# haotiansun14/rl-rep

Measured on NVIDIA B200. Metric: agent updates/sec, higher is better.
Workload: dtype tf32

## Files before the change

include/rlrep_b200.h:

```cpp
#ifndef RLREP_B200_H_
#define RLREP_B200_H_

#include <stddef.h>
#include <stdint.h>

#ifdef __cplusplus
extern "C" {
#endif

#if defined(__GNUC__)
#define RLREP_EXPORT __attribute__((visibility("default")))
#else
#define RLREP_EXPORT
#endif

#define RLREP_ABI_VERSION 3

RLREP_EXPORT int rlrep_abi_version(void);
RLREP_EXPORT const char* rlrep_last_error(void);


enum { RLREP_ACT_NONE = 0, RLREP_ACT_ELU = 1, RLREP_ACT_RELU = 2, RLREP_ACT_TANH = 3, RLREP_ACT_SIN = 4 };
enum {
  RLREP_DACT_NONE = 0,
  RLREP_DACT_ELU_OUT = 1,
  RLREP_DACT_RELU_OUT = 2,
  RLREP_DACT_TANH_OUT = 3,
  RLREP_DACT_COS_PRE = 4
};

typedef struct rlrep_epilogue {
  const float* bias_dev;
  const float* r1_u_dev;
  const float* r1_v_dev;
  const float* aux_dev;
  float* pre_out_dev;
  int ld_aux;
  int ld_pre;
  int act;
  int dact;
  int accumulate;
  float scale;
} rlrep_epilogue;

RLREP_EXPORT int rlrep_gemm(void* stream, int path, int M, int N, int K, const float* A_dev, int lda, int a_mn,
                            const float* A2_dev, int lda2, int K1, const float* B_dev, int ldb, int b_mn,
                            float* C_dev, int ldc, const rlrep_epilogue* epi, int bn, int split_k, float* ws_dev,
                            size_t ws_floats);

RLREP_EXPORT int rlrep_gemm_bench(void* stream, int path, int M, int N, int K, const float* A_dev, int lda, int a_mn,
                                  const float* B_dev, int ldb, int b_mn, float* C_dev, int ldc,
                                  const rlrep_epilogue* epi, int bn, int split_k, float* ws_dev, size_t ws_floats,
                                  int iters, float* ms_out, int* bn_out, int* split_out);

RLREP_EXPORT int rlrep_gemm_chain_begin(void);
RLREP_EXPORT int rlrep_gemm_chain_add(int M, int N, int K, const float* A_dev, int lda, int a_mn, const float* B_dev,
                                      int ldb, int b_mn, float* C_dev, int ldc, const rlrep_epilogue* epi);
RLREP_EXPORT int rlrep_gemm_chain_run(void* stream, int bn, int split_k, int iters, float* ms_out, int* levels_out);
RLREP_EXPORT int rlrep_gemm_chain_set_debug(unsigned long long* dev);

RLREP_EXPORT int rlrep_gemm_trace(unsigned long long* out16_host);
RLREP_EXPORT int rlrep_gemm_set_debug_buffer(unsigned long long* dev80);

typedef struct rlrep_ring rlrep_ring;

RLREP_EXPORT int rlrep_ring_create(int state_dim, int action_dim, long long capacity, rlrep_ring** out);
RLREP_EXPORT int rlrep_ring_destroy(rlrep_ring* ring);
RLREP_EXPORT int rlrep_ring_layout(const rlrep_ring* ring, int* record_floats, int* off_action, int* off_reward,
                                   int* off_done, int* off_next_state);
RLREP_EXPORT int rlrep_ring_state(const rlrep_ring* ring, long long* size, long long* ptr, long long* capacity);
RLREP_EXPORT int rlrep_ring_add_packed(rlrep_ring* ring, const float* rows_host, int n, void* stream);
RLREP_EXPORT int rlrep_ring_load(rlrep_ring* ring, const void* state_host, const void* action_host,
                                 const void* next_state_host, const void* reward_host, const void* done_host,
                                 long long n, int is_f64, void* stream);
RLREP_EXPORT int rlrep_ring_gather(rlrep_ring* ring, const int64_t* idx_host, int B, float* out_dev, void* stream);

typedef struct rlrep_pixring rlrep_pixring;
RLREP_EXPORT int rlrep_pixring_create(long long capacity, int frame_bytes, int action_dim, int frame_stack, int nstep,
                                      rlrep_pixring** out);
RLREP_EXPORT int rlrep_pixring_destroy(rlrep_pixring* ring);
RLREP_EXPORT int rlrep_pixring_write(rlrep_pixring* ring, long long slot, int copies, const unsigned char* frame_host,
                                     const float* action_host, float reward, float discount, int has_step);
RLREP_EXPORT int rlrep_pixring_flush(rlrep_pixring* ring);
RLREP_EXPORT int rlrep_pixring_gather(rlrep_pixring* ring, const int64_t* idx_host, int n, const float* discount_vec_host,
                                      float next_dis, unsigned char* obs_dev, float* act_dev, float* rew_dev, float* dis_dev,
                                      unsigned char* nobs_dev, unsigned char* sobs_dev);

typedef struct rlrep_agent rlrep_agent;

enum { RLREP_ALG_SAC = 0, RLREP_ALG_CTRLSAC = 1, RLREP_ALG_VLSAC = 2, RLREP_ALG_SPEDERSAC = 3, RLREP_ALG_DIFFSRSAC = 4 };
enum { RLREP_PRECISION_TF32 = 0, RLREP_PRECISION_FP32 = 1 };

typedef struct rlrep_agent_config {
  int alg;
  int state_dim, action_dim, batch_size;
  int hidden_dim, feature_dim, actor_hidden_dim;
  int feature_steps;
  double lr_critic, lr_feature, lr_actor, lr_alpha;
  float discount, tau, feature_tau;
  double alpha;
  int target_update_period, auto_entropy_tuning, use_feature_target;
  int precision;
  int use_cuda_graph;
  int phi_hidden_dim, phi_hidden_depth, mu_hidden_dim, mu_hidden_depth;
  int nabla_mu_hidden_dim, nabla_mu_hidden_depth, num_noise, num_noises;
  float sigma_scale_factor;
} rlrep_agent_config;

RLREP_EXPORT int rlrep_agent_create(const rlrep_agent_config* cfg, void* stream, rlrep_agent** out);

typedef struct rlrep_comm rlrep_comm;
RLREP_EXPORT int rlrep_comm_unique_id(unsigned char* out128);
RLREP_EXPORT int rlrep_comm_create(const unsigned char* id128, int rank, int world, rlrep_comm** out);
RLREP_EXPORT int rlrep_comm_destroy(rlrep_comm* comm);
RLREP_EXPORT int rlrep_comm_info(rlrep_comm* comm, int* rank, int* world, int* nccl_version, long long* collectives);
RLREP_EXPORT int rlrep_agent_create_sharded(const rlrep_agent_config* cfg, rlrep_comm* comm, void* stream,
                                            rlrep_agent** out);
RLREP_EXPORT int rlrep_agent_destroy(rlrep_agent* agent);

RLREP_EXPORT int rlrep_agent_num_tensors(rlrep_agent* agent, int* n);
RLREP_EXPORT int rlrep_agent_tensor_info(rlrep_agent* agent, int i, const char** name, float** ptr_dev, int* rows,
                                         int* cols);
RLREP_EXPORT int rlrep_agent_tensor_read(rlrep_agent* agent, int i, float* out_host);
RLREP_EXPORT int rlrep_agent_tensor_write(rlrep_agent* agent, int i, const float* in_host);
RLREP_EXPORT int rlrep_agent_sync_targets(rlrep_agent* agent);
RLREP_EXPORT int rlrep_agent_get_log_alpha(rlrep_agent* agent, double* log_alpha);
RLREP_EXPORT int rlrep_agent_set_log_alpha(rlrep_agent* agent, double log_alpha);
typedef struct rlrep_optim_state {
  int steps;
  long long t_feature, t_critic, t_actor, t_alpha;
  double log_alpha, log_alpha_m, log_alpha_v;
} rlrep_optim_state;
RLREP_EXPORT int rlrep_agent_get_optim_state(rlrep_agent* agent, rlrep_optim_state* out);
RLREP_EXPORT int rlrep_agent_set_optim_state(rlrep_agent* agent, const rlrep_optim_state* in);
RLREP_EXPORT int rlrep_agent_get_steps(rlrep_agent* agent, int* steps);

RLREP_EXPORT int rlrep_agent_train_counts(rlrep_agent* agent, int* n_idx, int* n_eps, int* n_metrics);
RLREP_EXPORT const char* rlrep_agent_metric_name(rlrep_agent* agent, int i);
RLREP_EXPORT int rlrep_agent_train(rlrep_agent* agent, rlrep_ring* ring, const int64_t* idx_host, int n_idx,
                                   const float* eps_host, int n_eps, float* metrics_host, int n_metrics);
RLREP_EXPORT int rlrep_agent_act(rlrep_agent* agent, const float* state_host, const float* eps_host,
// ... 132 lines not shown
```

rlrep_b200/_lib.py:

```python
from __future__ import annotations

import ctypes as C
from pathlib import Path

_HERE = Path(__file__).resolve().parent
LIB_PATH = _HERE / "librlrep_b200.so"


class RlrepError(RuntimeError):
    pass


class OptimState(C.Structure):
    _fields_ = [("steps", C.c_int), ("t_feature", C.c_longlong), ("t_critic", C.c_longlong), ("t_actor", C.c_longlong),
                ("t_alpha", C.c_longlong), ("log_alpha", C.c_double), ("log_alpha_m", C.c_double),
                ("log_alpha_v", C.c_double)]


class AgentConfig(C.Structure):
    _fields_ = [
        ("alg", C.c_int), ("state_dim", C.c_int), ("action_dim", C.c_int), ("batch_size", C.c_int),
        ("hidden_dim", C.c_int), ("feature_dim", C.c_int), ("actor_hidden_dim", C.c_int), ("feature_steps", C.c_int),
        ("lr_critic", C.c_double), ("lr_feature", C.c_double), ("lr_actor", C.c_double), ("lr_alpha", C.c_double),
        ("discount", C.c_float), ("tau", C.c_float), ("feature_tau", C.c_float), ("alpha", C.c_double),
        ("target_update_period", C.c_int), ("auto_entropy_tuning", C.c_int), ("use_feature_target", C.c_int),
        ("precision", C.c_int), ("use_cuda_graph", C.c_int),
        ("phi_hidden_dim", C.c_int), ("phi_hidden_depth", C.c_int), ("mu_hidden_dim", C.c_int),
        ("mu_hidden_depth", C.c_int), ("nabla_mu_hidden_dim", C.c_int), ("nabla_mu_hidden_depth", C.c_int),
        ("num_noise", C.c_int), ("num_noises", C.c_int), ("sigma_scale_factor", C.c_float),
    ]


ALG = {"sac": 0, "ctrlsac": 1, "vlsac": 2, "spedersac": 3, "diffsrsac": 4}
PRECISION = {"tf32": 0, "fp32": 1}


class Epilogue(C.Structure):
    _fields_ = [
        ("bias", C.c_void_p), ("r1_u", C.c_void_p), ("r1_v", C.c_void_p), ("aux", C.c_void_p),
        ("pre_out", C.c_void_p), ("ld_aux", C.c_int), ("ld_pre", C.c_int), ("act", C.c_int),
        ("dact", C.c_int), ("accumulate", C.c_int), ("scale", C.c_float),
    ]


ACT = {"none": 0, "elu": 1, "relu": 2, "tanh": 3, "sin": 4}
DACT = {"none": 0, "elu_out": 1, "relu_out": 2, "tanh_out": 3, "cos_pre": 4}

_lib = None


def load() -> C.CDLL:
    global _lib
    if _lib is not None:
        return _lib
    if not LIB_PATH.exists():
        raise RlrepError(
            f"{LIB_PATH} not found: build it with `python -m rlrep_b200.build` (needs nvcc). "
            "rlrep_b200 has no CPU or PyTorch fallback.")
    lib = C.CDLL(str(LIB_PATH))
    lib.rlrep_last_error.restype = C.c_char_p
    lib.rlrep_abi_version.restype = C.c_int
    _declare(lib)
    _lib = lib
    return lib


def _declare(lib: C.CDLL) -> None:
    vp, i, f, sz = C.c_void_p, C.c_int, C.c_float, C.c_size_t
    sigs = {
        "rlrep_gemm": [vp, i, i, i, i, vp, i, i, vp, i, i, vp, i, i, vp, i, C.POINTER(Epilogue), i, i, vp, sz],
        "rlrep_gemm_bench": [vp, i, i, i, i, vp, i, i, vp, i, i, vp, i, C.POINTER(Epilogue), i, i, vp, sz, i,
                             C.POINTER(C.c_float), C.POINTER(C.c_int), C.POINTER(C.c_int)],
        "rlrep_gemm_trace": [vp],
        "rlrep_gemm_chain_begin": [],
        "rlrep_gemm_chain_set_debug": [vp],
        "rlrep_gemm_chain_add": [i, i, i, vp, i, i, vp, i, i, vp, i, C.POINTER(Epilogue)],
        "rlrep_gemm_chain_run": [vp, i, i, i, C.POINTER(C.c_float), C.POINTER(C.c_int)],
        "rlrep_ring_create": [i, i, C.c_longlong, C.POINTER(vp)],
        "rlrep_ring_destroy": [vp],
        "rlrep_ring_layout": [vp] + [C.POINTER(i)] * 5,
        "rlrep_ring_state": [vp] + [C.POINTER(C.c_longlong)] * 3,
        "rlrep_ring_add_packed": [vp, vp, i, vp],
        "rlrep_ring_load": [vp, vp, vp, vp, vp, vp, C.c_longlong, i, vp],
        "rlrep_ring_gather": [vp, vp, i, vp, vp],
        "rlrep_agent_create": [C.POINTER(AgentConfig), vp, C.POINTER(vp)],
        "rlrep_agent_destroy": [vp],
        "rlrep_conv_encoder_create": [i, i, i, i, vp, C.POINTER(vp)],
        "rlrep_conv_encoder_destroy": [vp],
        "rlrep_conv_encoder_read": [vp, i, i, vp],
        "rlrep_conv_encoder_write": [vp, i, i, vp],
        "rlrep_conv_encoder_forward": [vp, vp, vp, vp],
        "rlrep_conv_encoder_backward": [vp, vp],
        "rlrep_conv_encoder_feature_dim": [vp, C.POINTER(i)],
        "rlrep_conv_encoder_forward_pitched": [vp, vp, vp, vp, i, i],
        "rlrep_conv_encoder_backward_pitched": [vp, vp, i],
        "rlrep_conv_encoder_read_map": [vp, i, i, vp],
        "rlrep_conv_decoder_create": [i, i, i, vp, C.POINTER(vp)],
        "rlrep_conv_decoder_destroy": [vp],
        "rlrep_conv_decoder_read": [vp, i, i, vp],
        "rlrep_conv_decoder_write": [vp, i, i, vp],
        "rlrep_conv_decoder_forward": [vp, vp, i],
        "rlrep_conv_decoder_l1_loss": [vp, vp, f, vp],
        "rlrep_conv_decoder_mse_sum_loss": [vp, vp, vp, f, vp],
        "rlrep_conv_decoder_backward": [vp, vp, i],
        "rlrep_conv_decoder_read_map": [vp, i, i, vp],
        "rlrep_drq_create": [vp, vp, C.POINTER(vp)],
        "rlrep_drq_destroy": [vp],
        "rlrep_drq_num_tensors": [vp, C.POINTER(i)],
        "rlrep_drq_tensor_info": [vp, i, C.POINTER(C.c_char_p), C.POINTER(vp), C.POINTER(i), C.POINTER(i)],
        "rlrep_drq_tensor_read": [vp, i, vp],
        "rlrep_drq_tensor_write": [vp, i, vp],
        "rlrep_drq_sync_targets": [vp],
        "rlrep_drq_update": [vp, vp, vp, vp, vp, vp, vp, vp, C.c_float, vp],
        "rlrep_drq_last_launches": [vp, C.POINTER(i)],
        "rlrep_drq_act": [vp, vp, vp, C.c_float, vp],
        "rlrep_drq_act_batch": [vp, vp, vp, C.c_float, i, vp],
        "rlrep_drq_update_resident": [vp, i, C.c_float, C.POINTER(C.c_float)],
        "rlrep_drq_profile_update": [vp, C.c_float, i, C.POINTER(C.c_char_p), C.POINTER(C.c_float), C.POINTER(C.c_double),
                                     C.POINTER(C.c_double), C.POINTER(i)],
        "rlrep_gemm_set_debug_buffer": [vp],
        "rlrep_ldiff_create": [vp, vp, C.POINTER(vp)],
        "rlrep_ldiff_destroy": [vp],
        "rlrep_ldiff_num_tensors": [vp, C.POINTER(i)],
        "rlrep_ldiff_tensor_info": [vp, i, C.POINTER(C.c_char_p), C.POINTER(vp), C.POINTER(i), C.POINTER(i)],
        "rlrep_ldiff_tensor_read": [vp, i, vp],
        "rlrep_ldiff_tensor_write": [vp, i, vp],
        "rlrep_ldiff_sync_targets": [vp],
        "rlrep_ldiff_update": [vp, vp, vp],
        "rlrep_ldiff_update_resident": [vp, i, C.c_float, C.POINTER(C.c_float)],
        "rlrep_ldiff_profile_update": [vp, C.c_float, i, C.POINTER(C.c_char_p), C.POINTER(C.c_float),
                                       C.POINTER(C.c_double), C.POINTER(C.c_double), C.POINTER(i)],
        "rlrep_ldiff_last_launches": [vp, C.POINTER(i)],
        "rlrep_mulv_create": [vp, vp, C.POINTER(vp)],
        "rlrep_mulv_destroy": [vp],
        "rlrep_mulv_num_tensors": [vp, C.POINTER(i)],
        "rlrep_mulv_tensor_info": [vp, i, C.POINTER(C.c_char_p), C.POINTER(vp), C.POINTER(i), C.POINTER(i)],
        "rlrep_mulv_tensor_read": [vp, i, vp],
        "rlrep_mulv_tensor_write": [vp, i, vp],
        "rlrep_mulv_sync_targets": [vp],
        "rlrep_mulv_update": [vp, vp, vp, vp, vp, vp, vp, vp, vp, vp, vp, C.c_float, vp],
        "rlrep_mulv_last_launches": [vp, C.POINTER(i)],
        "rlrep_mulv_act": [vp, vp, vp, C.c_float, vp],
        "rlrep_mulv_act_batch": [vp, vp, vp, C.c_float, i, vp],
        "rlrep_mulv_update_resident": [vp, i, C.c_float, C.POINTER(C.c_float)],
        "rlrep_mulv_profile_update": [vp, C.c_float, i, C.POINTER(C.c_char_p), C.POINTER(C.c_float), C.POINTER(C.c_double),
                                      C.POINTER(C.c_double), C.POINTER(i)],
        "rlrep_comm_unique_id": [vp],
        "rlrep_comm_create": [vp, i, i, C.POINTER(vp)],
        "rlrep_comm_destroy": [vp],
        "rlrep_comm_info": [vp, C.POINTER(i), C.POINTER(i), C.POINTER(i), C.POINTER(C.c_longlong)],
        "rlrep_agent_create_sharded": [C.POINTER(AgentConfig), vp, vp, C.POINTER(vp)],
        "rlrep_agent_num_tensors": [vp, C.POINTER(i)],
        "rlrep_agent_tensor_info": [vp, i, C.POINTER(C.c_char_p), C.POINTER(vp), C.POINTER(i), C.POINTER(i)],
        "rlrep_agent_tensor_read": [vp, i, vp],
        "rlrep_agent_tensor_write": [vp, i, vp],
        "rlrep_agent_sync_targets": [vp],
        "rlrep_agent_get_log_alpha": [vp, C.POINTER(C.c_double)],
        "rlrep_agent_set_log_alpha": [vp, C.c_double],
        "rlrep_agent_get_steps": [vp, C.POINTER(i)],
        "rlrep_agent_get_optim_state": [vp, C.POINTER(OptimState)],
        "rlrep_agent_set_optim_state": [vp, C.POINTER(OptimState)],
        "rlrep_agent_train_counts": [vp, C.POINTER(i), C.POINTER(i), C.POINTER(i)],
        "rlrep_agent_train": [vp, vp, vp, i, vp, i, vp, i],
        "rlrep_agent_act": [vp, vp, vp, vp],
        "rlrep_pixring_create": [C.c_longlong, i, i, i, i, C.POINTER(vp)],
        "rlrep_pixring_destroy": [vp],
        "rlrep_pixring_write": [vp, C.c_longlong, i, vp, vp, C.c_float, C.c_float, i],
        "rlrep_pixring_flush": [vp],
        "rlrep_pixring_gather": [vp, vp, i, vp, C.c_float, vp, vp, vp, vp, vp, vp],
        "rlrep_agent_act_batch": [vp, vp, vp, i, vp],
        "rlrep_agent_last_launches": [vp, C.POINTER(i)],
        "rlrep_agent_graph_stats": [vp, C.POINTER(i), C.POINTER(i)],
        "rlrep_agent_train_resident": [vp, vp, vp, vp, i, C.POINTER(C.c_float)],
        "rlrep_agent_profile_train": [vp, vp, vp, vp, i, C.POINTER(C.c_char_p), C.POINTER(C.c_float),
                                      C.POINTER(C.c_double), C.POINTER(C.c_double), C.POINTER(i)],
    }
    lib.rlrep_agent_metric_name.argtypes = [vp, i]
    lib.rlrep_agent_metric_name.restype = C.c_char_p
    for name, argtypes in sigs.items():
        fn = getattr(lib, name)
        fn.argtypes = argtypes
        fn.restype = C.c_int


def check(rc: int) -> None:
    if rc != 0:
        msg = load().rlrep_last_error()
        raise RlrepError(msg.decode() if msg else f"rlrep call failed with code {rc}")


def current_stream_ptr() -> int:
    import torch
    return torch.cuda.current_stream().cuda_stream


def make_epilogue(bias=None, r1=None, aux=None, pre_out=None, act="none", dact="none", accumulate=False,
                  scale=1.0) -> Epilogue:
    e = Epilogue()
    e.bias = bias.data_ptr() if bias is not None else None
    if r1 is not None:
        e.r1_u, e.r1_v = r1[0].data_ptr(), r1[1].data_ptr()
    if aux is not None:
        e.aux, e.ld_aux = aux.data_ptr(), aux.stride(0)
    if pre_out is not None:
        e.pre_out, e.ld_pre = pre_out.data_ptr(), pre_out.stride(0)
    e.act, e.dact = ACT[act], DACT[dact]
    e.accumulate = int(accumulate)
    e.scale = scale
    return e


def gemm(A, B, C_out, *, a_mn=False, b_mn=False, path="tc", epi: Epilogue | None = None, A2=None, bn=0, split_k=0,
         ws=None):
    lib = load()
    M = A.shape[1] if a_mn else A.shape[0]
    K = A.shape[0] if a_mn else A.shape[1]
    N = B.shape[1] if b_mn else B.shape[0]
    K1 = K
    if A2 is not None:
        K += A2.shape[1]
    assert (B.shape[0] if b_mn else B.shape[1]) == K
    epi = epi or make_epilogue()
    rc = lib.rlrep_gemm(current_stream_ptr(), 0 if path == "tc" else 1, M, N, K, A.data_ptr(), A.stride(0), int(a_mn),
                        A2.data_ptr() if A2 is not None else None, A2.stride(0) if A2 is not None else 0, K1,
                        B.data_ptr(), B.stride(0), int(b_mn), C_out.data_ptr(), C_out.stride(0), C.byref(epi), bn,
                        split_k, ws.data_ptr() if ws is not None else None, ws.numel() if ws is not None else 0)
    check(rc)
    return C_out


def gemm_chain(specs, *, bn=0, split_k=0, iters=1):
    lib = load()
    check(lib.rlrep_gemm_chain_begin())
    keep = []
    for A, B, C_out, kw in specs:
        a_mn, b_mn = bool(kw.get("a_mn", False)), bool(kw.get("b_mn", False))
        M = A.shape[1] if a_mn else A.shape[0]
        K = A.shape[0] if a_mn else A.shape[1]
        N = B.shape[1] if b_mn else B.shape[0]
        assert (B.shape[0] if b_mn else B.shape[1]) == K
        epi = kw.get("epi") or make_epilogue()
        keep.append(epi)
        check(lib.rlrep_gemm_chain_add(M, N, K, A.data_ptr(), A.stride(0), int(a_mn), B.data_ptr(), B.stride(0), int(b_mn),
                                       C_out.data_ptr(), C_out.stride(0), C.byref(epi)))
    ms, levels = C.c_float(), C.c_int()
    check(lib.rlrep_gemm_chain_run(current_stream_ptr(), bn, split_k, iters, C.byref(ms), C.byref(levels)))
    return ms.value, levels.value


def gemm_bench(A, B, C_out, *, a_mn=False, b_mn=False, path="tc", epi=None, bn=0, split_k=0, ws=None, iters=50):
    lib = load()
    M = A.shape[1] if a_mn else A.shape[0]
    K = A.shape[0] if a_mn else A.shape[1]
    N = B.shape[1] if b_mn else B.shape[0]
    epi = epi or make_epilogue()
    ms, bno, so = C.c_float(), C.c_int(), C.c_int()
    rc = lib.rlrep_gemm_bench(current_stream_ptr(), 0 if path == "tc" else 1, M, N, K, A.data_ptr(), A.stride(0),
                              int(a_mn), B.data_ptr(), B.stride(0), int(b_mn), C_out.data_ptr(), C_out.stride(0),
                              C.byref(epi), bn, split_k, ws.data_ptr() if ws is not None else None,
                              ws.numel() if ws is not None else 0, iters, C.byref(ms), C.byref(bno), C.byref(so))
    check(rc)
    return ms.value, bno.value, so.value
```

rlrep_b200/csrc/agent.cuh:

```cuda
#pragma once
#include <cuda_runtime.h>

#include <cstdint>
#include <cstring>
#include <functional>
#include <memory>
#include <string>
#include <unordered_map>
#include <vector>

#include "common.cuh"
#include "gemm.cuh"
#include "gemm_chain.cuh"
#include "kernels.cuh"

namespace rlrep {

class DeviceArena {
 public:
  DeviceArena() = default;
  DeviceArena(const DeviceArena&) = delete;
  DeviceArena& operator=(const DeviceArena&) = delete;
  ~DeviceArena() { release(); }
  template <typename T>
// ... 91 lines not shown
inline int round_up32(int x) { return (x + 31) & ~31; }

inline LinearSlot add_linear(ParamGroup& g, const std::string& name, int out, int in, bool pad = true) {
  LinearSlot s;
  s.out = out;
  s.in = in;
  s.ld = pad ? round_up32(in) : in;
  s.out_alloc = pad ? round_up32(out) : out;
  s.w_off = g.add(name + ".weight", out, in, s.ld, s.out_alloc);
  s.b_off = g.add(name + ".bias", out, 1, 1, s.out_alloc);
  return s;
}

inline LinearSlot add_stacked(ParamGroup& g, const std::string& a, int out_a, const std::string& b, int out_b, int in) {
  RLREP_CHECK(in % 32 == 0, "stacked heads need an input width that is a multiple of 32");
  LinearSlot s;
  s.out = out_a + out_b;
  s.in = in;
  s.ld = in;
  s.out_alloc = round_up32(s.out);
  s.w_off = g.add(a + ".weight", out_a, in);
  g.add(b + ".weight", out_b, in, in, s.out_alloc - out_a);
  s.b_off = g.add(a + ".bias", out_a, 1, 1, out_a, true);
  g.add(b + ".bias", out_b, 1, 1, s.out_alloc - out_a, true);
  g.align4();
  return s;
}

struct RecordLayout {
  int R, off_a, off_r, off_d, off_s2;
  static RecordLayout of(int S, int A) {
    RecordLayout l;
    l.off_a = S;
    l.off_r = S + A;
    l.off_d = S + A + 1;
    l.off_s2 = (S + A + 2 + 3) & ~3;
    l.R = (l.off_s2 + S + 3) & ~3;
    return l;
  }
};

class Ring {
 public:
  Ring(int state_dim, int action_dim, long long capacity);
  ~Ring();
  Ring(const Ring&) = delete;
  Ring& operator=(const Ring&) = delete;

  int S, A, R;
  int off_a, off_r, off_d, off_s2;
  long long capacity, size = 0, ptr = 0;
  float* data = nullptr;
  const unsigned long long generation;

  void add_packed(const float* rows_host, int n, cudaStream_t s);
  void load_columns(const void* state, const void* action, const void* next_state, const void* reward,
                    const void* done, long long n, int is_f64, cudaStream_t s);
  void gather_from_host_idx(const long long* idx_host, int B, float* out_dev, cudaStream_t s);

 private:
  float* stage_host_ = nullptr;
  float* stage_dev_ = nullptr;
  long long* idx_host_ = nullptr;
  long long* idx_dev_ = nullptr;
  size_t stage_rows_ = 0;
  int idx_cap_ = 0;
};

enum Precision : int { PREC_TF32 = 0, PREC_FP32 = 1 };

class GemmRunner {
 public:
  void init(Precision prec, size_t ws_floats);
  ~GemmRunner();
  void run(const GemmArgs& a, cudaStream_t s);
  bool run_compact(GemmArgs a, int wp, int ho, cudaStream_t s);
  bool compact_supported(GemmArgs a, int wp, int ho);
  void set_sm_share(double share) { sm_share_ = share; }

  bool chains_enabled() const { return prec_ == PREC_TF32; }
  void begin_chain(cudaStream_t s);
  void end_chain();
  bool recording() const { return recording_; }

 private:
  void flush_chain();
  bool recording_ = false;
  cudaStream_t chain_stream_ = nullptr;
  std::vector<GemmArgs> pending_;
  std::vector<std::unique_ptr<GemmChain>> chains_;
  Precision prec_ = PREC_TF32;
  double sm_share_ = 1.0;
  float* ws_ = nullptr;
  size_t ws_floats_ = 0;
  float* kg_ws_ = nullptr;
  size_t kg_ws_floats_ = 0;
  std::unordered_map<std::string, TcGemmPlan> plans_;
};

struct Mat {
  const float* p = nullptr;
  int ld = 0;
};
void linear_fwd(GemmRunner& g, cudaStream_t s, int rows, Mat x, const Linear& l, int act, float* y, int ldy,
                Mat x2 = Mat(), int k1 = 0, float* pre_out = nullptr);
void linear_dgrad(GemmRunner& g, cudaStream_t s, int rows, Mat dy, const Linear& l, int dact, Mat aux, float* dx,
                  int lddx, int col0 = 0, int n_cols = -1);
void linear_wgrad(GemmRunner& g, cudaStream_t s, int rows, Mat dy, Mat x, const Linear& l, Mat x2 = Mat(), int k1 = 0,
                  bool bias_grad = true);
inline ColJob bias_job(int rows, Mat dy, const Linear& l) {
  ColJob j;
  j.X = dy.p; j.ld = dy.ld; j.rows = rows; j.cols = l.out; j.u = nullptr; j.out = l.db;
  return j;
}

class GraphReplay {
 public:
  ~GraphReplay() { reset(); }
  void reset();
  void run(cudaStream_t s, bool enabled, const std::function<void()>& body);
  bool captured() const { return exec_ != nullptr; }
  bool stats(int* kernel_nodes, int* programmatic_edges) const;

 private:
  int calls_ = 0;
  cudaGraph_t graph_ = nullptr;
  cudaGraphExec_t exec_ = nullptr;
};

struct AgentConfig {
  int alg = 0;
  int state_dim = 0, action_dim = 0, batch = 256;
  int hidden_dim = 256, feature_dim = 256, actor_hidden_dim = 256;
  int k_feat = 0;
  double lr = 3e-4, lr_feat = 1e-4, lr_actor = 1e-4, lr_alpha = 1e-4;
  float discount = 0.99f, tau = 0.005f, feature_tau = 0.005f;
  double alpha0 = 0.1;
  int target_update_period = 2, learn_alpha = 1, use_feature_target = 1;
  int precision = PREC_TF32;
  int use_graph = 1;
  int phi_hidden_dim = 0, phi_hidden_depth = 0, mu_hidden_dim = 0, mu_hidden_depth = 0;
  int nabla_hidden_dim = 0, nabla_hidden_depth = 0, num_noise = 20, num_noises = 1000;
  float sigma_scale = 0.449f;
};

class Agent {
 public:
  virtual ~Agent() = default;
  virtual void train(Ring& ring, const long long* idx_host, int n_idx, const float* eps_host, int n_eps,
                     float* metrics_host, int n_metrics) = 0;
  virtual float train_resident(Ring& ring, const long long* idx_host, const float* eps_host, int n_steps) = 0;
  virtual std::vector<ProfileEntry> profile_train(Ring& ring, const long long* idx_host, const float* eps_host) = 0;
  virtual int idx_per_train() const = 0;
  virtual int eps_per_train() const = 0;
  virtual const std::vector<std::string>& metric_names() const = 0;
  virtual std::vector<ParamGroup*> groups() = 0;
  virtual void act(const float* state_host, const float* eps_host, float* action_host) = 0;
  virtual void act_batch(const float* states_host, const float* eps_host, int rows, float* actions_host) = 0;
  virtual void sync_targets_from_params() = 0;
  virtual bool graph_stats(int* kernel_nodes, int* programmatic_edges) const = 0;

  AgentConfig cfg;
  cudaStream_t stream = nullptr;
  Control* ctl = nullptr;
  int last_launches = 0;
};

std::unique_ptr<Agent> make_sac_agent(const AgentConfig& cfg, cudaStream_t s);
std::unique_ptr<Agent> make_ctrlsac_agent(const AgentConfig& cfg, cudaStream_t s);
std::unique_ptr<Agent> make_vlsac_agent(const AgentConfig& cfg, cudaStream_t s);
std::unique_ptr<Agent> make_spedersac_agent(const AgentConfig& cfg, cudaStream_t s);
std::unique_ptr<Agent> make_diffsrsac_agent(const AgentConfig& cfg, cudaStream_t s);
// ... 5 lines not shown
```

rlrep_b200/csrc/agent_ctrlsac.cu:

```cuda
#include "agent_base.cuh"

namespace rlrep {

namespace {

class CtrlSacAgent final : public SacBase {
 public:
  CtrlSacAgent(const AgentConfig& c, cudaStream_t s) : SacBase(c, s) {
    H_ = c.hidden_dim;
    D_ = c.feature_dim;
    K_ = c.k_feat;
    RLREP_CHECK(K_ >= 1 && K_ <= kMaxFeatureSteps, "extra_feature_steps out of range");
    const RecordLayout probe_layout = RecordLayout::of(S_, A_);
    off_r_ = probe_layout.off_r;
    off_d_ = probe_layout.off_d;
    off_s2_ = probe_layout.off_s2;
    plan_common(K_ * B_, 2 * B_ * A_, probe_layout.R);

    feat_g_.name = "feature";
    p1_ = add_linear(feat_g_, "phi.l1", H_, S_ + A_);
    p2_ = add_linear(feat_g_, "phi.l2", H_, H_);
    p3_ = add_linear(feat_g_, "phi.l3", D_, H_);
    feat_g_.n_target = feat_g_.n;
    feat_g_.target_prefix_from = "phi.";
// ... 167 lines not shown
      gemm_.run(a, s1);
    }
    wait_for(w1, mark(s1));
    gemm_.set_sm_share(wshare);
    linear_wgrad(gemm_, w1, B_, Mat{dzmu_, D_}, Mat{g2_, H_}, n3, Mat(), 0, false);
    gemm_.set_sm_share(share);
    linear_dgrad(gemm_, s1, B_, Mat{dzmu_, D_}, n3, DACT_ELU_OUT, Mat{g2_, H_}, dg2_, H_);
    wait_for(w1, mark(s1));
    gemm_.set_sm_share(wshare);
    linear_wgrad(gemm_, w1, B_, Mat{dg2_, H_}, Mat{g1_, H_}, n2, Mat(), 0, false);
    gemm_.set_sm_share(share);
    linear_dgrad(gemm_, s1, B_, Mat{dg2_, H_}, n2, DACT_ELU_OUT, Mat{g1_, H_}, dg1_, H_);
    linear_wgrad(gemm_, s1, B_, Mat{dg1_, H_}, s2(), n1, Mat(), 0, false);
    wait_for(w1, mark(s1));
    {
      ColJob jobs[3] = {bias_job(B_, Mat{dzmu_, D_}, n3), bias_job(B_, Mat{dg2_, H_}, n2),
                        bias_job(B_, Mat{dg1_, H_}, n1)};
      launch_colreduce_multi(jobs, 3, w1);
    }
    join_aux(0, s0);
    join_aux(1, s0);
    join();
    launch_adam_polyak(feat_g_.p, feat_g_.g, feat_g_.m, feat_g_.v, feat_g_.n, &ctl->feat[k],
                       cfg.use_feature_target ? feat_g_.target : nullptr, feat_g_.n_target, cfg.feature_tau, nullptr,
                       s0);
  }

  void feature_step_chained(int k, Ring& ring) {
    const Linear l1 = p1_.view(feat_g_), l2 = p2_.view(feat_g_), l3 = p3_.view(feat_g_);
    const Linear n1 = m1_.view(feat_g_), n2 = m2_.view(feat_g_), n3 = m3_.view(feat_g_);
    const Linear th = th_.view(feat_g_);
    const float inv_b = 1.f / (float)B_;
    cudaStream_t s0 = stream;
    launch_gather(ring.data, R_ / 4, idx_dev_ + (size_t)k * B_, B_, batch_, s0);
    gemm_.begin_chain(s0);
    phi_forward(s0, sa(), Mat(), 0, zphi_, h1_, h2_);
    linear_fwd(gemm_, s0, B_, s2(), n1, ACT_ELU, g1_, H_);
    linear_fwd(gemm_, s0, B_, Mat{g1_, H_}, n2, ACT_ELU, g2_, H_);
    linear_fwd(gemm_, s0, B_, Mat{g2_, H_}, n3, ACT_TANH, zmu_, D_);
    {
      GemmArgs a;
      a.M = B_; a.N = B_; a.K = D_;
      a.A = zphi_; a.lda = D_;
      a.B = zmu_; a.ldb = D_;
      a.C = logits_; a.ldc = B_;
      gemm_.run(a, s0);
    }
    if (k == K_ - 1) {
      actor_trunk(s2(), 1, s0);
      actor_trunk(Mat{batch_, R_}, 0, s0);
    }
    gemm_.end_chain();
    launch_contrastive_head(logits_, B_, B_, B_, 0, inv_b, zphi_, D_, D_, th.W, th.b, reward(), R_, loss_rows_, rpred_, drp_,
                            metrics_dev_ + 0, head_ctr_, s0);
    gemm_.begin_chain(s0);
    {
      GemmArgs a;
      a.M = B_; a.N = D_; a.K = B_;
      a.A = logits_; a.lda = B_;
      a.B = zmu_; a.ldb = D_; a.b_mn = true;
      a.C = dzphi_; a.ldc = D_;
      a.epi.r1_u = drp_; a.epi.r1_v = th.W;
      gemm_.run(a, s0);
    }
    {
      GemmArgs a;
      a.M = B_; a.N = D_; a.K = B_;
      a.A = logits_; a.lda = B_; a.a_mn = true;
      a.B = zphi_; a.ldb = D_; a.b_mn = true;
      a.C = dzmu_; a.ldc = D_;
      a.epi.dact = DACT_TANH_OUT; a.epi.aux = zmu_; a.epi.ld_aux = D_;
      gemm_.run(a, s0);
    }
    linear_dgrad(gemm_, s0, B_, Mat{dzphi_, D_}, l3, DACT_ELU_OUT, Mat{h2_, H_}, dh2_, H_);
    linear_dgrad(gemm_, s0, B_, Mat{dzmu_, D_}, n3, DACT_ELU_OUT, Mat{g2_, H_}, dg2_, H_);
    linear_wgrad(gemm_, s0, B_, Mat{dzphi_, D_}, Mat{h2_, H_}, l3, Mat(), 0, false);
    linear_wgrad(gemm_, s0, B_, Mat{dzmu_, D_}, Mat{g2_, H_}, n3, Mat(), 0, false);
    linear_dgrad(gemm_, s0, B_, Mat{dh2_, H_}, l2, DACT_ELU_OUT, Mat{h1_, H_}, dh1_, H_);
    linear_dgrad(gemm_, s0, B_, Mat{dg2_, H_}, n2, DACT_ELU_OUT, Mat{g1_, H_}, dg1_, H_);
    linear_wgrad(gemm_, s0, B_, Mat{dh2_, H_}, Mat{h1_, H_}, l2, Mat(), 0, false);
    linear_wgrad(gemm_, s0, B_, Mat{dg2_, H_}, Mat{g1_, H_}, n2, Mat(), 0, false);
    linear_wgrad(gemm_, s0, B_, Mat{dh1_, H_}, sa(), l1, Mat(), 0, false);
    linear_wgrad(gemm_, s0, B_, Mat{dg1_, H_}, s2(), n1, Mat(), 0, false);
    gemm_.end_chain();
    {
      ColJob jobs[8] = {bias_job(B_, Mat{dzphi_, D_}, l3), bias_job(B_, Mat{dh2_, H_}, l2),
                        bias_job(B_, Mat{dh1_, H_}, l1), ColJob{zphi_, drp_, th.dW, D_, B_, D_},
                        ColJob{drp_, nullptr, th.db, 1, B_, 1},
                        bias_job(B_, Mat{dzmu_, D_}, n3), bias_job(B_, Mat{dg2_, H_}, n2),
                        bias_job(B_, Mat{dg1_, H_}, n1)};
      launch_colreduce_multi(jobs, 8, s0);
    }
    launch_adam_polyak(feat_g_.p, feat_g_.g, feat_g_.m, feat_g_.v, feat_g_.n, &ctl->feat[k],
                       cfg.use_feature_target ? feat_g_.target : nullptr, feat_g_.n_target, cfg.feature_tau, nullptr,
                       s0);
  }

  void critic_step_chained() {
    cudaStream_t s0 = stream;
    const float* eps_next = eps_dev_;
    const float* eps_pi = eps_dev_ + (size_t)B_ * A_;
    const Linear l14t = c14_.view(crit_g_, true), l14 = c14_.view(crit_g_), l2 = c2_.view(crit_g_), l5 = c5_.view(crit_g_);
    const Linear l2t = c2_.view(crit_g_, true), l5t = c5_.view(crit_g_, true);
    actor_sample_cat_pair(s2(), eps_next, logp2_, Mat{batch_, R_}, eps_pi, s0);
    const Mat s2a{cat_next_, LDSA_}, spi{cat_pi_, LDSA_};
    gemm_.begin_chain(s0);
    phi_forward(s0, s2a, Mat(), 0, zmu_, h1_, h2_);
    linear_fwd(gemm_, s0, B_, Mat{zmu_, D_}, l14t, ACT_ELU, hid_t_, 2 * H_);
    phi_forward(s0, sa(), Mat(), 0, zphi_, hb1_, hb2_);
    linear_fwd(gemm_, s0, B_, Mat{zphi_, D_}, l14, ACT_ELU, hid_, 2 * H_);
    phi_forward(s0, spi, Mat(), 0, zpi_, hc1_, hc2_);
    gemm_.end_chain();
    {
      CriticHeadArgs a;
      a.hid_t = hid_t_; a.hid = hid_; a.ldh = 2 * H_; a.H = H_; a.B = B_;
      a.w2t = l2t.W; a.b2t = l2t.b; a.w5t = l5t.W; a.b5t = l5t.b;
      a.w2 = l2.W; a.b2 = l2.b; a.w5 = l5.W; a.b5 = l5.b;
      a.reward = reward(); a.done = done(); a.ld_rd = R_;
      a.logp2 = logp2_; a.gamma = cfg.discount; a.c = ctl;
      a.nq1 = nq1_; a.nq2 = nq2_; a.q1 = q1_; a.q2 = q2_; a.dq1 = dq1_; a.dq2 = dq2_;
      a.dhid = dhid_; a.ld_dh = 2 * H_;
      a.metrics = metrics_dev_ + 3;
      a.counter = head_ctr_ + 1;
      launch_critic_td_head(a, s0);
    }
    {
      ColJob jobs[5] = {ColJob{hid_, dq1_, l2.dW, 2 * H_, B_, H_}, ColJob{dq1_, nullptr, l2.db, 1, B_, 1},
                        ColJob{hid_ + H_, dq2_, l5.dW, 2 * H_, B_, H_}, ColJob{dq2_, nullptr, l5.db, 1, B_, 1},
                        bias_job(B_, Mat{dhid_, 2 * H_}, l14)};
      launch_colreduce_multi(jobs, 5, s0);
    }
    linear_wgrad(gemm_, s0, B_, Mat{dhid_, 2 * H_}, Mat{zphi_, D_}, l14, Mat(), 0, false);
    launch_adam_polyak(crit_g_.p, crit_g_.g, crit_g_.m, crit_g_.v, crit_g_.n, &ctl->critic, crit_g_.target,
                       crit_g_.n_target, cfg.tau, &ctl->polyak_critic, s0);
  }

  void actor_step_chained() {
    const float* eps = eps_dev_ + (size_t)B_ * A_;
    const Linear l14 = c14_.view(crit_g_);
    const Linear l1 = p1_.view(feat_g_), l2 = p2_.view(feat_g_), l3 = p3_.view(feat_g_);
    {
      const Linear c2 = c2_.view(crit_g_), c5 = c5_.view(crit_g_);
      linear_fwd(gemm_, stream, B_, Mat{zpi_, D_}, l14, ACT_ELU, hid_, 2 * H_);
      ActorHeadArgs a;
      a.hid = hid_; a.ldh = 2 * H_; a.H = H_; a.B = B_;
      a.w2 = c2.W; a.b2 = c2.b; a.w5 = c5.W; a.b5 = c5.b;
      a.logp = logp_; a.target_entropy = (float)(-A_); a.learn_alpha = cfg.learn_alpha; a.c = ctl;
      a.q1 = q1_; a.q2 = q2_; a.dq1 = dq1_; a.dq2 = dq2_;
      a.dhid = dhid_; a.ld_dh = 2 * H_;
      a.dlogp_scalar = dlogp_;
      a.metrics = metrics_dev_ + 7;
      a.counter = head_ctr_ + 2;
      launch_actor_head(a, stream);
    }
    gemm_.begin_chain(stream);
    linear_dgrad(gemm_, stream, B_, Mat{dhid_, 2 * H_}, l14, DACT_NONE, Mat(), dzphi_, D_);
    linear_dgrad(gemm_, stream, B_, Mat{dzphi_, D_}, l3, DACT_ELU_OUT, Mat{hc2_, H_}, dh2_, H_);
    linear_dgrad(gemm_, stream, B_, Mat{dh2_, H_}, l2, DACT_ELU_OUT, Mat{hc1_, H_}, dh1_, H_);
    dgrad_to_action(Mat{dh1_, H_}, l1);
    gemm_.end_chain();
    actor_backward_chained(Mat{batch_, R_}, eps);
    actor_adam();
  }

  void critic_forward(cudaStream_t s, const float* z, bool target, float* hid, float* q1, float* q2) {
    const Linear l14 = c14_.view(crit_g_, target), l2 = c2_.view(crit_g_, target), l5 = c5_.view(crit_g_, target);
    linear_fwd(gemm_, s, B_, Mat{z, D_}, l14, ACT_ELU, hid, 2 * H_);
    launch_rowdot_pair(RowDotJob{hid, l2.W, l2.b, q1, 2 * H_, H_}, RowDotJob{hid + H_, l5.W, l5.b, q2, 2 * H_, H_}, B_, s);
  }
  void critic_heads_backward_to_hidden() {
    const Linear l2 = c2_.view(crit_g_), l5 = c5_.view(crit_g_);
    launch_outer_dact(dq1_, l2.W, B_, H_, hid_, 2 * H_, DACT_ELU_OUT, dhid_, 2 * H_, stream);
    launch_outer_dact(dq2_, l5.W, B_, H_, hid_ + H_, 2 * H_, DACT_ELU_OUT, dhid_ + H_, 2 * H_, stream);
  }

  void critic_step() {
    const float* eps = eps_dev_;
    cudaStream_t s0 = stream, s1 = side();
// ... 66 lines not shown
```

rlrep_b200/csrc/capi.cu:

```cuda
#include <algorithm>
#include <cmath>
#include <memory>
#include <string>
#include <vector>

#include "agent.cuh"
#include "gemm_chain.cuh"
#include "comm.cuh"
#include "common.cuh"
#include "conv.cuh"
#include "deconv.cuh"
#include "drq.cuh"
#include "layout.cuh"
#include "mulv.cuh"
#include "pixel_replay.cuh"
#include "ldiffsr.cuh"
#include "gemm.cuh"
#include "rlrep_b200.h"

namespace rlrep {
namespace {
thread_local std::string g_last_error;
}
void set_last_error(const std::string& msg) { g_last_error = msg; }
// ... 37 lines not shown
  int prev = -1;
  explicit DeviceGuard(int want) {
    if (want < 0) return;
    int cur = 0;
    if (cudaGetDevice(&cur) == cudaSuccess && cur != want && cudaSetDevice(want) == cudaSuccess) prev = cur;
  }
  ~DeviceGuard() {
    if (prev >= 0) cudaSetDevice(prev);
  }
};
#define RLREP_API_BEGIN_ON(h) RLREP_API_BEGIN DeviceGuard _device_guard((h) != nullptr ? (h)->device : -1);

struct rlrep_ring {
  int device = current_device();
  std::unique_ptr<Ring> impl;
};

struct rlrep_comm {
  int device = current_device();
  std::unique_ptr<Comm> impl;
};

struct TensorRef {
  std::string name;
  float* ptr;
  int rows, cols, ld;
};

struct rlrep_agent {
  int device = current_device();
  std::unique_ptr<Agent> impl;
  std::vector<TensorRef> tensors;
  cudaStream_t owned_stream = nullptr;
};

static void index_tensors(rlrep_agent* a) {
  a->tensors.clear();
  for (ParamGroup* g : a->impl->groups()) {
    for (const ParamTensor& t : g->tensors) a->tensors.push_back({t.name, g->p + t.offset, t.rows, t.cols, t.ld});
    if (g->m && g->v)
      for (const ParamTensor& t : g->tensors) {
        a->tensors.push_back({"optim.m/" + t.name, g->m + t.offset, t.rows, t.cols, t.ld});
        a->tensors.push_back({"optim.v/" + t.name, g->v + t.offset, t.rows, t.cols, t.ld});
      }
    if (g->target) {
      for (const ParamTensor& t : g->tensors) {
        if (t.offset >= g->n_target) continue;
        if (t.name.compare(0, g->target_prefix_from.size(), g->target_prefix_from) != 0) continue;
        a->tensors.push_back({g->target_prefix_to + t.name.substr(g->target_prefix_from.size()), g->target + t.offset,
                              t.rows, t.cols, t.ld});
      }
    }
  }
}

extern "C" {

int rlrep_abi_version(void) { return RLREP_ABI_VERSION; }
const char* rlrep_last_error(void) { return get_last_error(); }

int rlrep_gemm(void* stream, int path, int M, int N, int K, const float* A, int lda, int a_mn, const float* A2,
               int lda2, int K1, const float* B, int ldb, int b_mn, float* C, int ldc, const rlrep_epilogue* epi,
               int bn, int split_k, float* ws, size_t ws_floats) {
  RLREP_API_BEGIN
  GemmArgs g;
  g.M = M; g.N = N; g.K = K;
  g.A = A; g.lda = lda; g.a_mn = a_mn != 0;
  g.A2 = A2; g.lda2 = lda2; g.K1 = K1;
  g.B = B; g.ldb = ldb; g.b_mn = b_mn != 0;
  g.C = C; g.ldc = ldc;
  g.epi = to_epilogue(epi);
  cudaStream_t st = static_cast<cudaStream_t>(stream);
  if (path == 0) {
    TcGemmPlan p = make_tc_plan(g, bn, split_k, ws, ws_floats);
    launch_tc(p, st);
  } else {
    launch_simt(g, st);
  }
  RLREP_API_END
}

namespace {
thread_local std::vector<GemmArgs> g_chain_seq;
}

int rlrep_gemm_chain_set_debug(unsigned long long* dev) {
  RLREP_API_BEGIN
  set_chain_debug_buffer(dev);
  RLREP_API_END
}

int rlrep_gemm_chain_begin(void) {
  RLREP_API_BEGIN
  g_chain_seq.clear();
  RLREP_API_END
}

int rlrep_gemm_chain_add(int M, int N, int K, const float* A, int lda, int a_mn, const float* B, int ldb, int b_mn,
                         float* C, int ldc, const rlrep_epilogue* epi) {
  RLREP_API_BEGIN
  GemmArgs g;
  g.M = M; g.N = N; g.K = K;
  g.A = A; g.lda = lda; g.a_mn = a_mn != 0;
  g.B = B; g.ldb = ldb; g.b_mn = b_mn != 0;
  g.C = C; g.ldc = ldc;
  g.epi = to_epilogue(epi);
  RLREP_CHECK(chain_eligible(g), "operands violate the tensor-core path's constraints (see rlrep_gemm, path 0)");
  g_chain_seq.push_back(g);
  RLREP_API_END
}

int rlrep_gemm_chain_run(void* stream, int bn, int split_k, int iters, float* ms_out, int* levels_out) {
  RLREP_API_BEGIN
  RLREP_CHECK(!g_chain_seq.empty() && iters >= 1, "empty chain");
  cudaStream_t st = static_cast<cudaStream_t>(stream);
  GemmChain chain;
  chain.build(g_chain_seq, bn, split_k);
  if (levels_out) *levels_out = chain.levels();
  cudaEvent_t e0, e1;
  RLREP_CUDA(cudaEventCreate(&e0));
  RLREP_CUDA(cudaEventCreate(&e1));
  chain.launch(st);
  RLREP_CUDA(cudaEventRecord(e0, st));
  for (int i = 1; i < iters; ++i) chain.launch(st);
  RLREP_CUDA(cudaEventRecord(e1, st));
  RLREP_CUDA(cudaStreamSynchronize(st));
  float ms = 0.f;
  RLREP_CUDA(cudaEventElapsedTime(&ms, e0, e1));
  cudaEventDestroy(e0);
  cudaEventDestroy(e1);
  if (ms_out) *ms_out = iters > 1 ? ms / (iters - 1) : 0.f;
  g_chain_seq.clear();
  RLREP_API_END
}

int rlrep_gemm_bench(void* stream, int path, int M, int N, int K, const float* A, int lda, int a_mn, const float* B,
                     int ldb, int b_mn, float* C, int ldc, const rlrep_epilogue* epi, int bn, int split_k, float* ws,
                     size_t ws_floats, int iters, float* ms_out, int* bn_out, int* split_out) {
  RLREP_API_BEGIN
  GemmArgs g;
  g.M = M; g.N = N; g.K = K;
  g.A = A; g.lda = lda; g.a_mn = a_mn != 0;
  g.B = B; g.ldb = ldb; g.b_mn = b_mn != 0;
  g.C = C; g.ldc = ldc;
  g.epi = to_epilogue(epi);
  cudaStream_t st = static_cast<cudaStream_t>(stream);
  cudaEvent_t e0, e1;
  RLREP_CUDA(cudaEventCreate(&e0));
  RLREP_CUDA(cudaEventCreate(&e1));
  TcGemmPlan p;
  if (path == 0) {
    p = make_tc_plan(g, bn, split_k, ws, ws_floats);
    if (bn_out) *bn_out = p.bn;
    if (split_out) *split_out = p.split_k;
  }
  auto launch_once = [&](cudaStream_t s) {
    if (path == 0) launch_tc(p, s);
    else if (path == 1) launch_simt(g, s);
    else if (path == 2) null_kernel<<<M, 128, 0, s>>>(C);
    else {
      cudaLaunchConfig_t cfg = {};
      cfg.gridDim = dim3(M);
      cfg.blockDim = dim3(128);
      cfg.stream = s;
      cudaLaunchAttribute at[1];
      at[0].id = cudaLaunchAttributeProgrammaticStreamSerialization;
      at[0].val.programmaticStreamSerializationAllowed = 1;
      cfg.attrs = at;
      cfg.numAttrs = 1;
      RLREP_CUDA(cudaLaunchKernelEx(&cfg, null_pdl_kernel, C));
    }
  };
  for (int i = 0; i < 3; ++i) launch_once(st);
  cudaStream_t cs;
  RLREP_CUDA(cudaStreamCreateWithFlags(&cs, cudaStreamNonBlocking));
  cudaGraph_t graph;
  cudaGraphExec_t exec;
  RLREP_CUDA(cudaStreamSynchronize(st));
  RLREP_CUDA(cudaStreamBeginCapture(cs, cudaStreamCaptureModeThreadLocal));
  for (int i = 0; i < iters; ++i) launch_once(cs);
  RLREP_CUDA(cudaStreamEndCapture(cs, &graph));
  RLREP_CUDA(cudaGraphInstantiate(&exec, graph, 0));
  RLREP_CUDA(cudaGraphLaunch(exec, cs));
  RLREP_CUDA(cudaEventRecord(e0, cs));
  RLREP_CUDA(cudaGraphLaunch(exec, cs));
  RLREP_CUDA(cudaEventRecord(e1, cs));
  RLREP_CUDA(cudaStreamSynchronize(cs));
  cudaGraphExecDestroy(exec);
  cudaGraphDestroy(graph);
  cudaStreamDestroy(cs);
  RLREP_CUDA(cudaEventSynchronize(e1));
  float ms = 0.f;
  RLREP_CUDA(cudaEventElapsedTime(&ms, e0, e1));
  *ms_out = ms / iters;
  cudaEventDestroy(e0);
  cudaEventDestroy(e1);
  RLREP_API_END
}

int rlrep_gemm_set_debug_buffer(unsigned long long* dev80) {
  RLREP_API_BEGIN
  set_gemm_debug_buffer(dev80);
  RLREP_API_END
}
int rlrep_gemm_trace(unsigned long long* out16_host) {
  RLREP_API_BEGIN
  RLREP_CUDA(cudaDeviceSynchronize());
  read_gemm_trace(out16_host);
  RLREP_API_END
}

int rlrep_ring_create(int state_dim, int action_dim, long long capacity, rlrep_ring** out) {
  RLREP_API_BEGIN
  RLREP_CHECK(out != nullptr, "null out pointer");
  std::unique_ptr<rlrep_ring> r(new rlrep_ring);
// ... 986 lines not shown
```

rlrep_b200/csrc/gemm_chain.cu:

```cuda
#include <algorithm>
#include <cmath>
#include <cstdlib>
#include <cstring>

#include "common.cuh"
#include "gemm_chain.cuh"
#include "ptx.cuh"

namespace rlrep {

namespace {

constexpr int kThreads = 320;
constexpr int kEpiWarps = 8;
constexpr int kStages = 6;
constexpr int kCW = 16;
constexpr int kTwPitch = kCW + 4;
constexpr int kMaxBn = 128;
constexpr int kBM = 128, kBK = 32;
constexpr int kABytes = kBM * kBK * 4;
constexpr int kStageBytes = kABytes + kMaxBn * kBK * 4;
constexpr int kTbufFloats = kEpiWarps * 32 * kTwPitch;
constexpr int kSub = 4, kCtrStride = 32;
constexpr int kDbgItems = 16, kDbgEvents = 10;
// ... 57 lines not shown
  const float e = __expf(n) - 1.f;
  const float r = n < -0.34657359f ? e : p;
  return x > 0.f ? x : r;
}

__device__ __forceinline__ bool aligned16(const void* p) { return (reinterpret_cast<uintptr_t>(p) & 15) == 0; }

__device__ __forceinline__ float chain_epilogue_scalar(const Epilogue& e, float acc, int m, int n, const float* cptr) {
  float v = acc * e.scale;
  if (e.r1_u) v = fmaf(__ldcg(e.r1_u + m), __ldcg(e.r1_v + n), v);
  if (e.bias) v += __ldg(e.bias + n);
  if (e.pre_out) e.pre_out[(size_t)m * e.ld_pre + n] = v;
  v = apply_act(v, e.act);
  if (e.dact != DACT_NONE) v *= apply_dact(__ldcg(e.aux + (size_t)m * e.ld_aux + n), e.dact);
  if (e.accumulate) v += __ldcg(cptr);
  return v;
}

struct ChunkOperands {
  float4 bias, r1v;
  float4 aux[4];
  float r1u[4];
};
__device__ __forceinline__ void chunk_prefetch(ChunkOperands& o, const Epilogue& epi, int M, int m_base, int gn0, int lane) {
  const int piece = lane & 3, rsub = lane >> 2;
  const int on = gn0 + 4 * piece;
  o.bias = make_float4(0.f, 0.f, 0.f, 0.f);
  o.r1v = make_float4(0.f, 0.f, 0.f, 0.f);
  if (epi.bias) o.bias = __ldg(reinterpret_cast<const float4*>(epi.bias + on));
  if (epi.r1_u) o.r1v = __ldcg(reinterpret_cast<const float4*>(epi.r1_v + on));
#pragma unroll
  for (int r4 = 0; r4 < 4; ++r4) {
    const int om = m_base + r4 * 8 + rsub;
    o.aux[r4] = make_float4(0.f, 0.f, 0.f, 0.f);
    o.r1u[r4] = 0.f;
    if (om < M) {
      if (epi.dact != DACT_NONE) o.aux[r4] = __ldcg(reinterpret_cast<const float4*>(epi.aux + (size_t)om * epi.ld_aux + on));
      if (epi.r1_u) o.r1u[r4] = __ldcg(epi.r1_u + om);
    }
  }
}

template <int ACT, int DACT>
__device__ __forceinline__ void chain_store_rows(const Epilogue& epi, const ChunkOperands& o, const float* tw,
                                                 float* __restrict__ C, int ldc, int M, int m_base, int gn0, int lane) {
  const int piece = lane & 3, rsub = lane >> 2;
  const int on = gn0 + 4 * piece;
#pragma unroll
  for (int r4 = 0; r4 < 4; ++r4) {
    const int r = r4 * 8 + rsub;
    const int om = m_base + r;
    if (om < M) {
      const float4 a4 = *reinterpret_cast<const float4*>(tw + r * kTwPitch + 4 * piece);
      float v[4] = {a4.x * epi.scale, a4.y * epi.scale, a4.z * epi.scale, a4.w * epi.scale};
      if (epi.r1_u) {
        const float u = o.r1u[r4];
        v[0] = fmaf(u, o.r1v.x, v[0]); v[1] = fmaf(u, o.r1v.y, v[1]); v[2] = fmaf(u, o.r1v.z, v[2]); v[3] = fmaf(u, o.r1v.w, v[3]);
      }
      v[0] += o.bias.x; v[1] += o.bias.y; v[2] += o.bias.z; v[3] += o.bias.w;
      if (epi.pre_out)
        *reinterpret_cast<float4*>(epi.pre_out + (size_t)om * epi.ld_pre + on) = make_float4(v[0], v[1], v[2], v[3]);
      if constexpr (ACT != ACT_NONE) {
#pragma unroll
        for (int e = 0; e < 4; ++e) v[e] = ACT == ACT_ELU ? elu_fast(v[e]) : apply_act(v[e], ACT < 0 ? epi.act : ACT);
      }
      if constexpr (DACT != DACT_NONE) {
        const int dact = DACT < 0 ? epi.dact : DACT;
        if (dact != DACT_NONE) {
          const float4 x = o.aux[r4];
          v[0] *= apply_dact(x.x, dact); v[1] *= apply_dact(x.y, dact); v[2] *= apply_dact(x.z, dact); v[3] *= apply_dact(x.w, dact);
        }
      }
      float4* cp = reinterpret_cast<float4*>(C + (size_t)om * ldc + on);
      if (epi.accumulate) {
        const float4 c0 = __ldcg(cp);
        v[0] += c0.x; v[1] += c0.y; v[2] += c0.z; v[3] += c0.w;
      }
      *cp = make_float4(v[0], v[1], v[2], v[3]);
    }
  }
}

__global__ void __launch_bounds__(kThreads, 1)
gemm_chain_kernel(const ChainGemmDesc* __restrict__ gemms, const ChainTask* __restrict__ tasks,
                  const int* __restrict__ task_begin, unsigned* __restrict__ done, unsigned* __restrict__ exit_ctr,
                  int n_gemms, unsigned long long* __restrict__ dbg) {
  auto stamp = [&](int item, int ev) {
    if (dbg != nullptr && item < kDbgItems) {
      unsigned long long t;
      asm volatile("mov.u64 %0, %%globaltimer;" : "=l"(t)::"memory");
      dbg[((size_t)blockIdx.x * kDbgItems + item) * kDbgEvents + ev] = t;
    }
  };
  if (threadIdx.x == 0) stamp(kDbgItems - 1, 2);
  extern __shared__ uint8_t smem_raw[];
  uint8_t* smem = reinterpret_cast<uint8_t*>((reinterpret_cast<uintptr_t>(smem_raw) + 1023) & ~uintptr_t(1023));
  uint64_t* full_bar = reinterpret_cast<uint64_t*>(smem + kStages * kStageBytes);
  uint64_t* empty_bar = full_bar + 8;
  uint64_t* acc_full = empty_bar + 8;
  uint64_t* acc_empty = acc_full + 2;
  uint32_t* tmem_slot = reinterpret_cast<uint32_t*>(acc_empty + 2);
  volatile unsigned* arrival = reinterpret_cast<volatile unsigned*>(tmem_slot + 1);
  float* tbuf = reinterpret_cast<float*>(smem + kStages * kStageBytes + 256);

  const int warp = threadIdx.x >> 5, lane = threadIdx.x & 31;
  const int t_begin = task_begin[blockIdx.x], t_end = task_begin[blockIdx.x + 1];

  if (threadIdx.x == 0) {
    for (int s = 0; s < kStages; ++s) {
      ptx::mbar_init(&full_bar[s], 1);
      ptx::mbar_init(&empty_bar[s], 1);
    }
    for (int a = 0; a < 2; ++a) {
      ptx::mbar_init(&acc_full[a], 1);
      ptx::mbar_init(&acc_empty[a], kEpiWarps);
    }
    ptx::fence_mbar_init();
  }
  if (warp == 1) {
    ptx::tmem_alloc(tmem_slot, 2 * kMaxBn);
    ptx::tmem_relinquish();
  }
  ptx::tc_fence_before_sync();
  __syncthreads();
  ptx::tc_fence_after_sync();
  const uint32_t tmem_base = *tmem_slot;
  ptx::pdl_wait();

  if (warp == 0) {
    if (lane == 0) {
      int it = 0, last_gemm = -1;
      for (int t = t_begin; t < t_end; ++t) {
        const ChainTask tk = tasks[t];
        const ChainGemmDesc* g = gemms + tk.gemm;
        const int n_deps = g->n_deps;
        const int bn = g->bn, a_mn = g->a_mn, b_mn = g->b_mn;
        const int m0 = (tk.tile % g->tiles_m) * kBM, n0 = (tk.tile / g->tiles_m) * bn;
        const int kb0 = tk.split * g->kb_per_split, kb1 = min(g->nkb, kb0 + g->kb_per_split);
        int dep_id[kChainMaxDeps], dep_tiles[kChainMaxDeps];
#pragma unroll
        for (int d = 0; d < kChainMaxDeps; ++d) {
          dep_id[d] = d < n_deps ? g->dep[d] : 0;
          dep_tiles[d] = d < n_deps ? (int)g->dep_target[d] : 0;
        }
        if (tk.gemm != last_gemm) {
          fence_tensormap_acquire(&g->tmA);
          fence_tensormap_acquire(&g->tmB);
          last_gemm = tk.gemm;
        }
        stamp(t - t_begin, 0);
        if (dbg != nullptr && t - t_begin < kDbgItems)
          dbg[((size_t)blockIdx.x * kDbgItems + (t - t_begin)) * kDbgEvents + 8] =
              (unsigned long long)tk.gemm | ((unsigned long long)tk.tile << 16) | ((unsigned long long)tk.split << 40);
#pragma unroll
        for (int d = 0; d < kChainMaxDeps; ++d)
          if (d < n_deps) wait_counter(done, dep_id[d], dep_tiles[d]);
        if (n_deps > 0) {
          fence_acquire_gpu();
          fence_proxy_async_global();
        }
        stamp(t - t_begin, 1);
        const uint32_t tx = kABytes + bn * kBK * 4;
        for (int kb = kb0; kb < kb1; ++kb, ++it) {
          const int s = it % kStages;
          ptx::mbar_wait(&empty_bar[s], ((it / kStages) & 1) ^ 1);
          ptx::mbar_arrive_expect_tx(&full_bar[s], tx);
          uint8_t* a_dst = smem + s * kStageBytes;
          uint8_t* b_dst = a_dst + kABytes;
          const int k0 = kb * kBK;
          if (!a_mn) ptx::tma_load_2d(a_dst, &g->tmA, &full_bar[s], k0, m0);
          else ptx::tma_load_3d(a_dst, &g->tmA, &full_bar[s], 0, k0, m0 / 32);
          if (!b_mn) ptx::tma_load_2d(b_dst, &g->tmB, &full_bar[s], k0, n0);
          else ptx::tma_load_3d(b_dst, &g->tmB, &full_bar[s], 0, k0, n0 / 32);
        }
        stamp(t - t_begin, 2);
      }
    }
  } else if (warp == 1) {
    if (ptx::elect_one()) {
      int it = 0, tc = 0;
      for (int t = t_begin; t < t_end; ++t, ++tc) {
        const ChainTask tk = tasks[t];
        const ChainGemmDesc* g = gemms + tk.gemm;
        const int bn = g->bn, a_mn = g->a_mn, b_mn = g->b_mn;
        const int kb0 = tk.split * g->kb_per_split, kb1 = min(g->nkb, kb0 + g->kb_per_split);
        const uint32_t idesc = ptx::make_idesc_tf32(kBM, bn, a_mn != 0, b_mn != 0);
        const int acc = tc & 1;
        ptx::mbar_wait(&acc_empty[acc], ((tc >> 1) & 1) ^ 1);
        ptx::tc_fence_after_sync();
        const uint32_t d_tmem = tmem_base + acc * kMaxBn;
        for (int kb = kb0; kb < kb1; ++kb, ++it) {
          const int s = it % kStages;
          ptx::mbar_wait(&full_bar[s], (it / kStages) & 1);
          if (kb == kb0) stamp(t - t_begin, 3);
          ptx::tc_fence_after_sync();
          const uint32_t a_addr = ptx::smem_u32(smem + s * kStageBytes);
          const uint32_t b_addr = a_addr + kABytes;
#pragma unroll
          for (int k = 0; k < kBK / 8; ++k) {
            const uint64_t adesc = a_mn ? ptx::make_smem_desc(a_addr + k * 1024, 4096, 512, 1)
                                        : ptx::make_smem_desc(a_addr + k * 32, 16, 1024, 2);
            const uint64_t bdesc = b_mn ? ptx::make_smem_desc(b_addr + k * 1024, 4096, 512, 1)
                                        : ptx::make_smem_desc(b_addr + k * 32, 16, 1024, 2);
            ptx::mma_tf32_ss(d_tmem, adesc, bdesc, idesc, (kb > kb0 || k > 0) ? 1u : 0u);
          }
          ptx::mma_commit(&empty_bar[s]);
        }
        ptx::mma_commit(&acc_full[acc]);
        stamp(t - t_begin, 4);
      }
    }
  } else {
    const int q = warp & 3, half = (warp - 2) >> 2;
    float* tw = tbuf + (warp - 2) * (32 * kTwPitch);
    int tc = 0;
    for (int t = t_begin; t < t_end; ++t, ++tc) {
      const ChainTask tk = tasks[t];
      const ChainGemmDesc* g = gemms + tk.gemm;
      const Epilogue epi = g->epi;
      const int bn = g->bn, M = g->M, N = g->N, ldc = g->ldc, split_k = g->split_k;
      float* __restrict__ C = g->C;
      float* __restrict__ ws = g->ws;
      unsigned* __restrict__ tile_ctr = g->tile_ctr;
      const int m0 = (tk.tile % g->tiles_m) * kBM, n0 = (tk.tile / g->tiles_m) * bn;
      const int chunks = bn / kCW;
      const int acc = tc & 1;
      const uint32_t t_acc = tmem_base + (static_cast<uint32_t>(32 * q) << 16) + acc * kMaxBn;
      const int row = 32 * q + lane;
      ptx::mbar_wait(&acc_full[acc], (tc >> 1) & 1);
      if (threadIdx.x == 64) stamp(t - t_begin, 5);
      ptx::tc_fence_after_sync();

      bool final = true;
      const size_t part_floats = (size_t)kBM * bn;
      float* ws_tile = split_k > 1 ? ws + (size_t)tk.tile * split_k * part_floats : nullptr;
      const bool dist = split_k > 1 && g->dist != 0;
      int c_first = half, c_step = 2;
      if (split_k > 1) {
        float* part = ws_tile + (size_t)tk.split * part_floats;
#pragma unroll 1
        for (int c = half; c < chunks; c += 2) {
          if (dist && c % split_k == tk.split) continue;
          uint32_t v[kCW];
          ptx::tmem_ld_32x32b_x16(t_acc + c * kCW, v);
          ptx::tmem_ld_wait();
#pragma unroll
          for (int j = 0; j < kCW / 4; ++j)
            __stcg(reinterpret_cast<float4*>(part + ((size_t)(c * (kCW / 4) + j) * kBM + row) * 4),
                   make_float4(__uint_as_float(v[4 * j]), __uint_as_float(v[4 * j + 1]), __uint_as_float(v[4 * j + 2]),
                               __uint_as_float(v[4 * j + 3])));
        }
        epilogue_bar();
        if (threadIdx.x == 64) {
          unsigned* ctr = tile_ctr + tk.tile;
          const unsigned old = atom_add_acq_rel(ctr, 1u);
          if (dist) {
            if (old + 1 < (unsigned)split_k) {
              unsigned long long t0 = 0;
              unsigned spins = 0;
              while (ld_relaxed(ctr) < (unsigned)split_k) {
                __nanosleep(20);
                if ((++spins & 0xfff) == 0) {
                  unsigned long long now;
                  asm volatile("mov.u64 %0, %%globaltimer;" : "=l"(now));
                  if (t0 == 0) t0 = now;
                  else if (now - t0 > 2000000000ull) __trap();
                }
              }
              fence_acquire_gpu();
            }
          } else if (old == (unsigned)(split_k - 1)) {
            *ctr = 0;
          }
          *arrival = old;
          stamp(t - t_begin, 6);
        }
        epilogue_bar();
        final = dist || *arrival == (unsigned)(split_k - 1);
        if (dist) {
          c_first = tk.split + split_k * half;
          c_step = 2 * split_k;
        }
      }
      if (final) {
        const bool use_aux = epi.dact != DACT_NONE;
        const bool vec_ok = (ldc & 3) == 0 && aligned16(C) && (N & 3) == 0 &&
                            (!use_aux || ((epi.ld_aux & 3) == 0 && aligned16(epi.aux))) &&
                            (!epi.pre_out || ((epi.ld_pre & 3) == 0 && aligned16(epi.pre_out))) &&
                            (!epi.bias || aligned16(epi.bias)) && (!epi.r1_v || aligned16(epi.r1_v));
#pragma unroll 1
        for (int c = c_first; c < chunks; c += c_step) {
          const int gn0 = n0 + c * kCW;
          const bool fast = vec_ok && gn0 + kCW <= N;
          ChunkOperands ops;
          if (fast) chunk_prefetch(ops, epi, M, m0 + 32 * q, gn0, lane);
          float a[kCW];
          if (split_k == 1) {
            uint32_t v[kCW];
            ptx::tmem_ld_32x32b_x16(t_acc + c * kCW, v);
            ptx::tmem_ld_wait();
// ... 3 lines not shown
            const float* base = ws_tile + ((size_t)(c * (kCW / 4)) * kBM + row) * 4;
            float4 nxt[kCW / 4];
            const int s_first = tk.split == 0 ? 1 : 0;
#pragma unroll
            for (int j = 0; j < kCW / 4; ++j)
              nxt[j] = __ldcg(reinterpret_cast<const float4*>(base + (size_t)s_first * part_floats + (size_t)j * kBM * 4));
#pragma unroll 1
            for (int s = 0; s < split_k; ++s) {
              if (s == tk.split) {
                uint32_t v[kCW];
                ptx::tmem_ld_32x32b_x16(t_acc + c * kCW, v);
                ptx::tmem_ld_wait();
                if (s == 0) {
#pragma unroll
                  for (int e = 0; e < kCW; ++e) a[e] = __uint_as_float(v[e]);
                } else {
#pragma unroll
                  for (int e = 0; e < kCW; ++e) a[e] += __uint_as_float(v[e]);
                }
                continue;
              }
              float4 cur[kCW / 4];
#pragma unroll
              for (int j = 0; j < kCW / 4; ++j) cur[j] = nxt[j];
              int s2 = s + 1;
              if (s2 == tk.split) ++s2;
              if (s2 < split_k) {
#pragma unroll
                for (int j = 0; j < kCW / 4; ++j)
                  nxt[j] = __ldcg(reinterpret_cast<const float4*>(base + (size_t)s2 * part_floats + (size_t)j * kBM * 4));
              }
              if (s == 0) {
#pragma unroll
                for (int j = 0; j < kCW / 4; ++j) { a[4 * j] = cur[j].x; a[4 * j + 1] = cur[j].y; a[4 * j + 2] = cur[j].z; a[4 * j + 3] = cur[j].w; }
              } else {
#pragma unroll
                for (int j = 0; j < kCW / 4; ++j) { a[4 * j] += cur[j].x; a[4 * j + 1] += cur[j].y; a[4 * j + 2] += cur[j].z; a[4 * j + 3] += cur[j].w; }
              }
            }
          }
#pragma unroll
          for (int j = 0; j < kCW / 4; ++j)
            *reinterpret_cast<float4*>(tw + lane * kTwPitch + 4 * j) = make_float4(a[4 * j], a[4 * j + 1], a[4 * j + 2], a[4 * j + 3]);
          __syncwarp();
          if (fast) {
#define RLREP_CSTORE(A, D) chain_store_rows<A, D>(epi, ops, tw, C, ldc, M, m0 + 32 * q, gn0, lane)
            RLREP_EPILOGUE_SWITCH(epi, RLREP_CSTORE);
#undef RLREP_CSTORE
          } else if (gn0 < N) {
            const int piece = lane & 3, rsub = lane >> 2;
#pragma unroll 1
            for (int r4 = 0; r4 < 4; ++r4) {
              const int r = r4 * 8 + rsub, om = m0 + 32 * q + r;
              if (om >= M) continue;
#pragma unroll 1
              for (int e = 0; e < 4; ++e) {
                const int on = gn0 + 4 * piece + e;
                if (on < N) {
                  float* cp = C + (size_t)om * ldc + on;
                  *cp = chain_epilogue_scalar(epi, tw[r * kTwPitch + 4 * piece + e], om, on, cp);
                }
              }
            }
          }
          __syncwarp();
        }
        if (threadIdx.x == 64) stamp(t - t_begin, 9);
        epilogue_bar();
        if (threadIdx.x == 64) {
          fence_proxy_async_global();
          const int pub = dist ? tk.tile * split_k + tk.split : tk.tile;
          red_release_add(done + ((size_t)tk.gemm * kSub + (pub % kSub)) * kCtrStride, 1u);
          stamp(t - t_begin, 7);
          if (dist) {
            unsigned* ctr = tile_ctr + tk.tile;
            if (atomicAdd(ctr, 1u) == (unsigned)(2 * split_k - 1)) *ctr = 0;
          }
        }
      }
      ptx::tc_fence_before_sync();
      __syncwarp();
      if (lane == 0) ptx::mbar_arrive(&acc_empty[acc]);
    }
  }
  ptx::pdl_launch_dependents();
  ptx::tc_fence_before_sync();
  __syncthreads();
  if (warp == 1) ptx::tmem_dealloc(tmem_base, 2 * kMaxBn);
  if (threadIdx.x == 0) {
    const unsigned old = atom_add_acq_rel(exit_ctr, 1u);
    if (old == gridDim.x - 1) {
      for (int i = 0; i < n_gemms * kSub; ++i) done[(size_t)i * kCtrStride] = 0;
      *exit_ctr = 0;
      __threadfence();
    }
    stamp(kDbgItems - 1, 3);
  }
}

struct Range {
  uintptr_t lo = 0, hi = 0;
  bool overlaps(const Range& o) const { return lo < o.hi && o.lo < hi && lo != hi && o.lo != o.hi; }
};
Range range_of(const float* p, long long rows, long long ld, long long cols) {
  Range r;
  if (p == nullptr || rows <= 0 || cols <= 0) return r;
  r.lo = reinterpret_cast<uintptr_t>(p);
  r.hi = r.lo + (size_t)((rows - 1) * ld + cols) * sizeof(float);
  return r;
}
struct Footprint {
  std::vector<Range> reads, writes;
};
Footprint footprint(const GemmArgs& a) {
  Footprint f;
  f.reads.push_back(a.a_mn ? range_of(a.A, a.K, a.lda, a.M) : range_of(a.A, a.M, a.lda, a.K));
  f.reads.push_back(a.b_mn ? range_of(a.B, a.K, a.ldb, a.N) : range_of(a.B, a.N, a.ldb, a.K));
  f.reads.push_back(range_of(a.epi.bias, 1, 0, a.N));
  f.reads.push_back(range_of(a.epi.r1_u, 1, 0, a.M));
  f.reads.push_back(range_of(a.epi.r1_v, 1, 0, a.N));
  if (a.epi.dact != DACT_NONE) f.reads.push_back(range_of(a.epi.aux, a.M, a.epi.ld_aux, a.N));
  f.writes.push_back(range_of(a.C, a.M, a.ldc, a.N));
  if (a.epi.accumulate) f.reads.push_back(f.writes.back());
  f.writes.push_back(range_of(a.epi.pre_out, a.M, a.epi.ld_pre, a.N));
  return f;
}
bool conflicts(const Footprint& earlier, const Footprint& later) {
  for (const Range& w : earlier.writes) {
    for (const Range& r : later.reads)
      if (w.overlaps(r)) return true;
    for (const Range& r : later.writes)
      if (w.overlaps(r)) return true;
  }
  for (const Range& w : later.writes)
    for (const Range& r : earlier.reads)
      if (w.overlaps(r)) return true;
  return false;
}

unsigned long long* g_chain_dbg = nullptr;

int env_int(const char* name, int dflt) {
  const char* e = std::getenv(name);
  return e ? std::atoi(e) : dflt;
}

bool dist_possible(int bn, int split) { return split > 1 && (bn / kCW) % split == 0; }
double plan_cost(int tiles, int nkb, int bn, int split, int share, bool dist) {
  const int kb_per = ceil_div(nkb, split);
  const double kb_bytes = kABytes + bn * kBK * 4;
  const double waves = std::ceil((double)tiles * split / share);
  const double stream = waves * kb_per * kb_bytes / 150e3;
  const double chip = (double)tiles * split * kb_per * kb_bytes / 12e6;
  if (dist) {
    return 1.5 + std::max(stream, chip) + waves * (0.25 * ceil_div(bn, 64) + 1.0 + 1.0 * ceil_div(bn / split, 64)) +
           0.1 * (split - 1);
  }
  double t = 1.5 + std::max(stream, chip) + waves * 1.0 * ceil_div(bn, 64);
  if (split > 1) t += 1.5 + 0.3 * (split - 1) * ceil_div(bn, 64);
  return t;
}

}

void set_chain_debug_buffer(unsigned long long* dev) { g_chain_dbg = dev; }

bool chain_eligible(const GemmArgs& a) {
  return tc_eligible(a) && a.conv_w == 0 && a.M >= 32 && a.N >= 32 && a.K >= 8;
}

GemmChain::~GemmChain() {
  if (dev_) cudaFree(dev_);
}

bool GemmChain::matches(const std::vector<GemmArgs>& seq) const {
  if (seq.size() != seq_.size()) return false;
  for (size_t i = 0; i < seq.size(); ++i) {
    const GemmArgs &x = seq[i], &y = seq_[i];
    if (x.M != y.M || x.N != y.N || x.K != y.K || x.A != y.A || x.B != y.B || x.C != y.C || x.lda != y.lda ||
        x.ldb != y.ldb || x.ldc != y.ldc || x.a_mn != y.a_mn || x.b_mn != y.b_mn || x.epi.bias != y.epi.bias ||
        x.epi.r1_u != y.epi.r1_u || x.epi.r1_v != y.epi.r1_v || x.epi.aux != y.epi.aux || x.epi.pre_out != y.epi.pre_out ||
        x.epi.ld_aux != y.epi.ld_aux || x.epi.ld_pre != y.epi.ld_pre || x.epi.act != y.epi.act || x.epi.dact != y.epi.dact ||
        x.epi.accumulate != y.epi.accumulate || x.epi.scale != y.epi.scale)
      return false;
  }
  return true;
}

void GemmChain::build(const std::vector<GemmArgs>& seq, int force_bn, int force_split) {
  RLREP_CHECK(dev_ == nullptr, "chain already built");
  RLREP_CHECK(!seq.empty(), "empty chain");
  const int n = (int)seq.size();
  for (const GemmArgs& a : seq) RLREP_CHECK(chain_eligible(a), "GEMM cannot be a member of a chain");
  seq_ = seq;
  int n_sm = kNumSMs;
  {
    int dev = 0;
    RLREP_CUDA(cudaGetDevice(&dev));
    RLREP_CUDA(cudaDeviceGetAttribute(&n_sm, cudaDevAttrMultiProcessorCount, dev));
  }
  static bool attr_set = false;
  if (!attr_set) {
    RLREP_CUDA(cudaFuncSetAttribute(gemm_chain_kernel, cudaFuncAttributeMaxDynamicSharedMemorySize, kSmemBytes));
    attr_set = true;
  }
  int per_sm = 0;
  RLREP_CUDA(cudaOccupancyMaxActiveBlocksPerMultiprocessor(&per_sm, gemm_chain_kernel, kThreads, kSmemBytes));
  RLREP_CHECK(per_sm >= 1, "chain kernel does not fit on an SM");
  const int n_cta = n_sm;

  std::vector<Footprint> fp(n);
  for (int i = 0; i < n; ++i) fp[i] = footprint(seq[i]);
  std::vector<std::vector<int>> deps(n);
  std::vector<std::vector<char>> reach(n, std::vector<char>(n, 0));
  std::vector<int> level(n, 0);
  for (int j = 0; j < n; ++j) {
    std::vector<int> direct;
    for (int i = 0; i < j; ++i)
      if (conflicts(fp[i], fp[j])) direct.push_back(i);
    for (int i : direct) {
      reach[j][i] = 1;
      for (int k = 0; k < n; ++k)
        if (reach[i][k]) reach[j][k] = 1;
    }
    for (int i : direct) {
      bool implied = false;
      for (int k : direct)
        if (k != i && reach[k][i]) implied = true;
      if (!implied) deps[j].push_back(i);
      level[j] = std::max(level[j], level[i] + 1);
    }
    RLREP_CHECK((int)deps[j].size() <= kChainMaxDeps, "a chain GEMM has too many direct dependencies");
  }
  levels_ = 1 + *std::max_element(level.begin(), level.end());

  std::vector<int> bn(n), split(n), share(n), first_cta(n), dist(n, 0);
  const int dist_mode = env_int("RLREP_CHAIN_DIST", 1);
  auto work_of = [&](int i) {
    return (double)ceil_div(seq[i].M, kBM) * ceil_div(seq[i].N, kMaxBn) * ceil_div(seq[i].K, kBK);
  };
  auto items_of = [&](int i) { return ceil_div(seq[i].M, kBM) * ceil_div(seq[i].N, bn[i]) * (dist[i] ? split[i] : 1); };
  for (int L = 0; L < levels_; ++L) {
    std::vector<int> members;
    for (int i = 0; i < n; ++i)
      if (level[i] == L) members.push_back(i);
    double total = 0.0;
    for (int i : members) total += work_of(i);
    int cursor = 0, seen = 0;
    for (int i : members) {
      const GemmArgs& a = seq[i];
      const int nkb = ceil_div(a.K, kBK);
      ++seen;
      int sh = std::max(4, (int)std::floor(n_cta * work_of(i) / total));
      if (seen == (int)members.size()) sh = std::max(sh, n_cta - cursor);
      sh = std::min(sh, n_cta);
      first_cta[i] = cursor % n_cta;
      cursor += sh;
      share[i] = sh;
      double best = 1e300;
      for (int cbn : {32, 64, 128}) {
        if (force_bn && cbn != force_bn) continue;
        if (!force_bn && cbn > 32 && cbn / 2 >= a.N) continue;
        const int tiles = ceil_div(a.M, kBM) * ceil_div(a.N, cbn);
        for (int s : {1, 2, 4, 8, 16}) {
          if (force_split && s != force_split) continue;
          if (s > 1 && (s - 1) * ceil_div(nkb, s) >= nkb) continue;
          for (int d = 0; d < 2; ++d) {
            if (d == 1 && (dist_mode == 0 || !dist_possible(cbn, s) || tiles * s > sh)) continue;
            if (d == 0 && dist_mode == 2 && dist_possible(cbn, s) && tiles * s <= sh) continue;
            const double c = plan_cost(tiles, nkb, cbn, s, sh, d == 1);
            if (c < best - 1e-9) {
              best = c;
              bn[i] = cbn;
              split[i] = s;
              dist[i] = d;
            }
          }
        }
      }
      if (best > 1e299) {
        bn[i] = force_bn ? force_bn : 32;
        split[i] = 1;
        dist[i] = 0;
      }
    }
  }

  std::vector<std::vector<ChainTask>> per_cta(n_cta);
  std::vector<int> order(n);
  for (int i = 0; i < n; ++i) order[i] = i;
  std::stable_sort(order.begin(), order.end(), [&](int x, int y) { return level[x] < level[y]; });
  size_t ws_floats = 0, ctr_count = 0;
  std::vector<size_t> ws_off(n, 0), ctr_off(n, 0);
  std::vector<ChainGemmDesc> descs(n);
  bytes_ = flops_ = 0.0;
  for (int i : order) {
    const GemmArgs& a = seq[i];
    const int tiles_m = ceil_div(a.M, kBM), tiles_n = ceil_div(a.N, bn[i]);
    const int tiles = tiles_m * tiles_n;
    int item = 0;
    for (int t = 0; t < tiles; ++t)
      for (int s = 0; s < split[i]; ++s, ++item)
        per_cta[(first_cta[i] + item % share[i]) % n_cta].push_back(ChainTask{i, t, s, 0});
    ChainGemmDesc& d = descs[i];
    std::memset(&d, 0, sizeof(d));
    d.tmA = make_operand_map(a.A, a.a_mn, a.M, a.K, a.lda, kBM);
    d.tmB = make_operand_map(a.B, a.b_mn, a.N, a.K, a.ldb, bn[i]);
    d.epi = a.epi;
    d.C = a.C;
    d.ldc = a.ldc; d.M = a.M; d.N = a.N; d.K = a.K;
    d.bn = bn[i]; d.a_mn = a.a_mn; d.b_mn = a.b_mn; d.nkb = ceil_div(a.K, kBK);
    d.split_k = split[i]; d.kb_per_split = ceil_div(d.nkb, split[i]);
    d.dist = dist[i];
    d.tiles_m = tiles_m; d.tiles_n = tiles_n;
    d.n_deps = (int)deps[i].size();
    for (int k = 0; k < d.n_deps; ++k) {
      const int j = deps[i][k];
      d.dep[k] = j;
      d.dep_target[k] = (unsigned)items_of(j);
    }
    ctr_off[i] = ctr_count;
    ctr_count += (size_t)tiles;
    if (split[i] > 1) {
      ws_off[i] = ws_floats;
      ws_floats += (size_t)tiles * split[i] * kBM * bn[i];
    }
    bytes_ += 4.0 * ((double)a.M * a.K + (double)a.N * a.K + (double)a.M * a.N);
    flops_ += 2.0 * a.M * a.N * a.K;
  }
  std::vector<ChainTask> tasks;
  std::vector<int> begin(n_cta + 1, 0);
  for (int c = 0; c < n_cta; ++c) {
    begin[c] = (int)tasks.size();
    tasks.insert(tasks.end(), per_cta[c].begin(), per_cta[c].end());
  }
  begin[n_cta] = (int)tasks.size();
  grid_ = n_cta;

  auto up = [](size_t x) { return (x + 255) & ~size_t(255); };
  const size_t o_desc = 0;
  const size_t o_tasks = up(o_desc + sizeof(ChainGemmDesc) * n);
  const size_t o_begin = up(o_tasks + sizeof(ChainTask) * tasks.size());
  const size_t o_done = up(o_begin + sizeof(int) * begin.size());
  const size_t o_exit = up(o_done + sizeof(unsigned) * n * kSub * kCtrStride);
  const size_t o_ctr = up(o_exit + sizeof(unsigned));
  const size_t o_ws = up(o_ctr + sizeof(unsigned) * ctr_count);
  const size_t total_bytes = o_ws + sizeof(float) * ws_floats + 256;
  RLREP_CUDA(cudaMalloc(&dev_, total_bytes));
  RLREP_CUDA(cudaMemset(dev_, 0, o_ws));
  char* base = static_cast<char*>(dev_);
  d_gemms_ = reinterpret_cast<ChainGemmDesc*>(base + o_desc);
  d_tasks_ = reinterpret_cast<ChainTask*>(base + o_tasks);
  d_task_begin_ = reinterpret_cast<int*>(base + o_begin);
  d_done_ = reinterpret_cast<unsigned*>(base + o_done);
  d_exit_ = reinterpret_cast<unsigned*>(base + o_exit);
  for (int i = 0; i < n; ++i) {
    descs[i].tile_ctr = reinterpret_cast<unsigned*>(base + o_ctr) + ctr_off[i];
    descs[i].ws = split[i] > 1 ? reinterpret_cast<float*>(base + o_ws) + ws_off[i] : nullptr;
  }
  RLREP_CUDA(cudaMemcpy(d_gemms_, descs.data(), sizeof(ChainGemmDesc) * n, cudaMemcpyHostToDevice));
  RLREP_CUDA(cudaMemcpy(d_tasks_, tasks.data(), sizeof(ChainTask) * tasks.size(), cudaMemcpyHostToDevice));
  RLREP_CUDA(cudaMemcpy(d_task_begin_, begin.data(), sizeof(int) * begin.size(), cudaMemcpyHostToDevice));
  RLREP_CUDA(cudaDeviceSynchronize());
  if (env_int("RLREP_CHAIN_VERBOSE", 0)) {
    std::fprintf(stderr, "rlrep chain: %d GEMMs, %d levels, %zu items, ws %.1f MB\n", n, levels_, tasks.size(),
                 ws_floats * 4 / 1e6);
    for (int i = 0; i < n; ++i)
      std::fprintf(stderr, "  [%d] L%d M=%d N=%d K=%d a_mn=%d b_mn=%d bn=%d split=%d%s share=%d deps=%d\n", i, level[i],
                   seq[i].M, seq[i].N, seq[i].K, (int)seq[i].a_mn, (int)seq[i].b_mn, bn[i], split[i],
                   dist[i] ? " (distributed)" : "", share[i], (int)deps[i].size());
  }
}

void GemmChain::launch(cudaStream_t stream) {
  RLREP_CHECK(dev_ != nullptr, "chain not built");
  cudaLaunchConfig_t cfg = {};
  cfg.gridDim = dim3(grid_);
  cfg.blockDim = dim3(kThreads);
  cfg.dynamicSmemBytes = kSmemBytes;
  cfg.stream = stream;
  cudaLaunchAttribute attr[2];
  attr[0].id = cudaLaunchAttributeCooperative;
  attr[0].val.cooperative = 1;
  attr[1] = pdl_attribute();
  cfg.attrs = attr;
  cfg.numAttrs = 2;
  RLREP_CUDA(cudaLaunchKernelEx(&cfg, gemm_chain_kernel, (const ChainGemmDesc*)d_gemms_, (const ChainTask*)d_tasks_,
                                (const int*)d_task_begin_, d_done_, d_exit_, (int)seq_.size(), g_chain_dbg));
  RLREP_LAUNCHED_W("gemm_chain", stream, bytes_, flops_);
}

}
```

rlrep_b200/csrc/gemm_chain.cuh:

```cuda
#pragma once
#include <vector>

#include "gemm.cuh"

namespace rlrep {

constexpr int kChainMaxDeps = 6;

struct alignas(128) ChainGemmDesc {
  CUtensorMap tmA;
  CUtensorMap tmB;
  Epilogue epi;
  int dist;
  float* C;
  float* ws;
  unsigned* tile_ctr;
  int ldc, M, N, K;
  int bn, a_mn, b_mn, nkb;
  int split_k, kb_per_split, tiles_m, tiles_n;
  int n_deps;
  int dep[kChainMaxDeps];
  unsigned dep_target[kChainMaxDeps];
};

struct ChainTask {
  int gemm, tile, split, pad;
};

class GemmChain {
 public:
  GemmChain() = default;
  GemmChain(const GemmChain&) = delete;
  GemmChain& operator=(const GemmChain&) = delete;
  ~GemmChain();
  bool matches(const std::vector<GemmArgs>& seq) const;
  void build(const std::vector<GemmArgs>& seq, int force_bn = 0, int force_split = 0);
  void launch(cudaStream_t stream);
  int size() const { return (int)seq_.size(); }
  int levels() const { return levels_; }

 private:
  std::vector<GemmArgs> seq_;
  void* dev_ = nullptr;
  ChainGemmDesc* d_gemms_ = nullptr;
  ChainTask* d_tasks_ = nullptr;
  int* d_task_begin_ = nullptr;
  unsigned* d_done_ = nullptr;
  unsigned* d_exit_ = nullptr;
  int grid_ = 0, levels_ = 0;
  double bytes_ = 0.0, flops_ = 0.0;
};

void set_chain_debug_buffer(unsigned long long* dev);

bool chain_eligible(const GemmArgs& a);

}
```

rlrep_b200/csrc/kernels.cu:

```cuda
#include <cmath>

#include "common.cuh"
#include "epilogue.cuh"
#include "kernels.cuh"
#include "ptx.cuh"
#include "reduce.cuh"

namespace rlrep {

namespace {

__device__ __forceinline__ AdamHyper adam_hyper(double lr, long long t) {
  const double bc1 = 1.0 - pow(0.9, (double)t);
  const double bc2 = 1.0 - pow(0.999, (double)t);
  AdamHyper h;
  h.step_size = (float)(lr / bc1);
  h.bc2_sqrt = (float)sqrt(bc2);
  return h;
}

__global__ void tick_kernel(Control* c, const TickParams p) {
  ptx::pdl_wait();
  ptx::pdl_launch_dependents();
  const int lane = threadIdx.x;
  if (blockIdx.x != 0 || lane >= 32) return;
  const long long t_feat = c->t_feat, t_critic = c->t_critic, t_actor = c->t_actor, t_alpha = c->t_alpha;
  const int steps = c->steps + 1;
  const double log_alpha = c->log_alpha;
  __syncwarp();
  const int k = p.k_feat;
  if (lane < k) c->feat[lane] = adam_hyper(p.lr_feat, t_feat + lane + 1);
  if (lane == k && p.critic_steps) c->critic = adam_hyper(p.lr_critic, t_critic + 1);
  if (lane == k + 1) c->actor = adam_hyper(p.lr_actor, t_actor + 1);
  if (lane == k + 2) c->alpha_step_size = p.lr_alpha / (1.0 - pow(0.9, (double)(t_alpha + 1)));
  if (lane == k + 3) c->alpha_bc2_sqrt = sqrt(1.0 - pow(0.999, (double)(t_alpha + 1)));
  if (lane == k + 4) {
    c->alpha = (float)exp(log_alpha);
    c->steps = steps;
    c->polyak_critic = (steps % p.period == 0) ? 1 : 0;
    c->t_feat = t_feat + k;
    if (p.critic_steps) c->t_critic = t_critic + 1;
    c->t_actor = t_actor + 1;
    c->t_alpha = t_alpha + 1;
  }
}

__global__ void gather_kernel(const float4* __restrict__ ring, int rec4, const long long* __restrict__ idx, int B,
                              float4* __restrict__ out) {
  ptx::pdl_wait();
  ptx::pdl_launch_dependents();
  const int total = B * rec4;
  for (int i = blockIdx.x * blockDim.x + threadIdx.x; i < total; i += gridDim.x * blockDim.x) {
    const int b = i / rec4, c = i - b * rec4;
    out[i] = __ldg(ring + (size_t)idx[b] * rec4 + c);
  }
}
__global__ void ring_write_kernel(float4* __restrict__ ring, int rec4, long long capacity, long long start,
                                  const float4* __restrict__ rows, int n) {
  const int total = n * rec4;
  for (int i = blockIdx.x * blockDim.x + threadIdx.x; i < total; i += gridDim.x * blockDim.x) {
    const int b = i / rec4, c = i - b * rec4;
    ring[(size_t)((start + b) % capacity) * rec4 + c] = rows[i];
  }
}

__global__ void __launch_bounds__(256) ce_rows_kernel(float* __restrict__ logits, int ld, int cols, int diag_off,
                                                      float inv_batch, float* __restrict__ loss_rows) {
  __shared__ float scratch[33];
  const int row = blockIdx.x;
  float* l = logits + (size_t)row * ld;
  float mx = -INFINITY;
  for (int j = threadIdx.x; j < cols; j += 256) mx = fmaxf(mx, l[j]);
  mx = block_max<256>(mx, scratch);
  float sum = 0.f;
  for (int j = threadIdx.x; j < cols; j += 256) sum += expf(l[j] - mx);
  sum = block_sum<256>(sum, scratch);
  const float lse = mx + logf(sum);
  const int dj = diag_off + row;
  if (threadIdx.x == 0) loss_rows[row] = lse - l[dj];
  __syncthreads();
  for (int j = threadIdx.x; j < cols; j += 256) {
    const float pr = expf(l[j] - lse);
// ... 570 lines not shown
  __syncthreads();
  head_backward_row(h, a.w2, a.w5, bc[0], bc[1], H, a.dhid + (size_t)row * a.ld_dh, tid);
  if (tid == 0) {
    __threadfence();
    last = atomicAdd(a.counter, 1u) == (unsigned)(a.B - 1);
  }
  __syncthreads();
  if (!last) return;
  __threadfence();
  Control* c = a.c;
  const float alpha = c->alpha, inv_b = 1.f / (float)a.B;
  float la = 0.f, ent = 0.f, raw = 0.f;
  for (int i = tid; i < a.B; i += 256) {
    const float v1 = __ldcg(a.q1 + i), v2 = __ldcg(a.q2 + i);
    la += alpha * a.logp[i] - fminf(v1, v2);
    ent += alpha * (-a.logp[i] - a.target_entropy);
    raw += -a.logp[i] - a.target_entropy;
  }
  la = block_sum<256>(la, scratch);
  ent = block_sum<256>(ent, scratch);
  raw = block_sum<256>(raw, scratch);
  if (tid == 0) {
    *a.dlogp_scalar = alpha * inv_b;
    a.metrics[0] = la * inv_b;
    a.metrics[1] = ent * inv_b;
    if (a.learn_alpha) {
      const double g = (double)(raw * inv_b) * exp(c->log_alpha);
      c->la_m = c->la_m + (1.0 - 0.9) * (g - c->la_m);
      c->la_v = c->la_v * 0.999 + (1.0 - 0.999) * g * g;
      const double denom = sqrt(c->la_v) / c->alpha_bc2_sqrt + 1e-8;
      c->log_alpha = c->log_alpha - c->alpha_step_size * (c->la_m / denom);
    }
    a.metrics[2] = (float)exp(c->log_alpha);
    *a.counter = 0;
  }
}

__global__ void __launch_bounds__(256) actor_loss_partial_kernel(const float* __restrict__ q1,
                                                                 const float* __restrict__ q2,
                                                                 const float* __restrict__ logp, int B, int norm_B,
                                                                 float target_entropy, const Control* __restrict__ c,
                                                                 float* __restrict__ dq1, float* __restrict__ dq2,
                                                                 float* __restrict__ dlogp_scalar,
                                                                 float* __restrict__ partial) {
  __shared__ float scratch[33];
  const float alpha = c->alpha;
  const float inv_b = 1.f / (float)norm_B;
  float la = 0.f, raw = 0.f;
  for (int i = threadIdx.x; i < B; i += 256) {
    const float a = q1[i], b = q2[i];
    la += alpha * logp[i] - fminf(a, b);
    raw += -logp[i] - target_entropy;
    const float g = -inv_b;
    dq1[i] = a < b ? g : (a == b ? 0.5f * g : 0.f);
    dq2[i] = b < a ? g : (a == b ? 0.5f * g : 0.f);
  }
  la = block_sum<256>(la, scratch);
  raw = block_sum<256>(raw, scratch);
  if (threadIdx.x == 0) {
    *dlogp_scalar = alpha * inv_b;
    partial[0] = la * inv_b;
    partial[1] = raw * inv_b;
  }
}
__global__ void alpha_step_kernel(const float* __restrict__ reduced, int learn_alpha, Control* c,
                                  float* __restrict__ metrics) {
  if (threadIdx.x != 0 || blockIdx.x != 0) return;
  metrics[0] = reduced[0];
  metrics[1] = c->alpha * reduced[1];
  if (learn_alpha) {
    const double g = (double)reduced[1] * exp(c->log_alpha);
    c->la_m = c->la_m + (1.0 - 0.9) * (g - c->la_m);
    c->la_v = c->la_v * 0.999 + (1.0 - 0.999) * g * g;
    const double denom = sqrt(c->la_v) / c->alpha_bc2_sqrt + 1e-8;
    c->log_alpha = c->log_alpha - c->alpha_step_size * (c->la_m / denom);
  }
  metrics[2] = (float)exp(c->log_alpha);
}
__global__ void mul_dact_kernel(float* __restrict__ x, const float* __restrict__ aux, size_t n, int dact) {
  for (size_t i = (size_t)blockIdx.x * blockDim.x + threadIdx.x; i < n; i += (size_t)gridDim.x * blockDim.x)
    x[i] *= apply_dact(aux[i], dact);
}

__device__ __forceinline__ float adam_elem(float& p, float g, float& m, float& v, float ss, float bc2s) {
  constexpr float w1 = (float)(1.0 - 0.9), b2 = 0.999f, w2 = (float)(1.0 - 0.999), eps = 1e-8f;
  m = fmaf(w1, g - m, m);
  v = fmaf(w2 * g, g, v * b2);
  const float denom = sqrtf(v) / bc2s + eps;
  p = p - ss * (m / denom);
  return p;
}

__global__ void __launch_bounds__(256) adam_polyak_kernel(float4* __restrict__ p, const float4* __restrict__ g,
                                                          float4* __restrict__ m, float4* __restrict__ v, size_t n4,
                                                          const AdamHyper* __restrict__ hyper,
                                                          float4* __restrict__ target, size_t n4_polyak, float tau,
                                                          const int* __restrict__ polyak_flag) {
  ptx::pdl_wait();
  ptx::pdl_launch_dependents();
  const float ss = hyper->step_size, bc2s = hyper->bc2_sqrt;
  const bool do_polyak = target != nullptr && (polyak_flag == nullptr || *polyak_flag != 0);
  const float omt = 1.f - tau;
  for (size_t i = (size_t)blockIdx.x * blockDim.x + threadIdx.x; i < n4; i += (size_t)gridDim.x * blockDim.x) {
    float4 pv = p[i], mv = __ldcs(m + i), vv = __ldcs(v + i);
    const float4 gv = __ldcs(g + i);
    adam_elem(pv.x, gv.x, mv.x, vv.x, ss, bc2s);
    adam_elem(pv.y, gv.y, mv.y, vv.y, ss, bc2s);
    adam_elem(pv.z, gv.z, mv.z, vv.z, ss, bc2s);
    adam_elem(pv.w, gv.w, mv.w, vv.w, ss, bc2s);
    p[i] = pv;
    __stcs(m + i, mv);
    __stcs(v + i, vv);
    if (do_polyak && i < n4_polyak) {
      float4 t = __ldcs(target + i);
      t.x = __fadd_rn(__fmul_rn(tau, pv.x), __fmul_rn(omt, t.x));
      t.y = __fadd_rn(__fmul_rn(tau, pv.y), __fmul_rn(omt, t.y));
      t.z = __fadd_rn(__fmul_rn(tau, pv.z), __fmul_rn(omt, t.z));
      t.w = __fadd_rn(__fmul_rn(tau, pv.w), __fmul_rn(omt, t.w));
      __stcs(target + i, t);
    }
  }
}

__global__ void __launch_bounds__(256) polyak_kernel(const float4* __restrict__ p, float4* __restrict__ target,
                                                     size_t n4, float tau, const int* __restrict__ polyak_flag) {
  if (polyak_flag != nullptr && *polyak_flag == 0) return;
  const float omt = 1.f - tau;
  for (size_t i = (size_t)blockIdx.x * blockDim.x + threadIdx.x; i < n4; i += (size_t)gridDim.x * blockDim.x) {
    const float4 pv = p[i];
    float4 t = target[i];
    t.x = __fadd_rn(__fmul_rn(tau, pv.x), __fmul_rn(omt, t.x));
    t.y = __fadd_rn(__fmul_rn(tau, pv.y), __fmul_rn(omt, t.y));
    t.z = __fadd_rn(__fmul_rn(tau, pv.z), __fmul_rn(omt, t.z));
    t.w = __fadd_rn(__fmul_rn(tau, pv.w), __fmul_rn(omt, t.w));
    target[i] = t;
  }
}

constexpr float kLogSigMin = -20.f, kLogSigMax = 2.f;
__device__ __forceinline__ float clamp_ls(float raw) { return fminf(fmaxf(raw, kLogSigMin), kLogSigMax); }
__device__ __forceinline__ float clamp_grad(float raw) { return (raw >= kLogSigMin && raw <= kLogSigMax) ? 1.f : 0.f; }

struct ColSegments {
  ColSegment s[3];
  int n;
};
__global__ void pack_columns_kernel(const float* __restrict__ in, int ld_in, float* __restrict__ out, int ld_out, int rows,
                                    const ColSegments segs, int width) {
  const size_t total = (size_t)rows * width;
  for (size_t i = (size_t)blockIdx.x * blockDim.x + threadIdx.x; i < total; i += (size_t)gridDim.x * blockDim.x) {
    const int r = (int)(i / width);
    int c = (int)(i - (size_t)r * width);
#pragma unroll
    for (int k = 0; k < 3; ++k) {
      if (k < segs.n) {
        if (c < segs.s[k].len) {
          out[(size_t)r * ld_out + segs.s[k].dst + c] = in[(size_t)r * ld_in + segs.s[k].src + c];
          break;
        }
        c -= segs.s[k].len;
      }
    }
  }
}

__global__ void vae_sample_kernel(const float* __restrict__ head, int ld_head, int B, int D, const float* __restrict__ eps,
                                  float* __restrict__ z) {
  const int total = B * D;
  for (int i = blockIdx.x * blockDim.x + threadIdx.x; i < total; i += gridDim.x * blockDim.x) {
    const int b = i / D, d = i - b * D;
    const float* h = head + (size_t)b * ld_head;
    z[i] = h[d] + eps[i] * expf(clamp_ls(h[D + d]));
  }
}

__global__ void __launch_bounds__(256) vae_recon_loss_kernel(const float* __restrict__ xr, int ld_xr,
                                                             const float* __restrict__ next_state,
                                                             const float* __restrict__ reward, int ld_rec, int B, int S,
                                                             float* __restrict__ dxr, float* __restrict__ partial) {
  __shared__ float scratch[33];
  const float gs = 1.f / ((float)B * (float)S), gr = 1.f / (float)B;
  float se_s = 0.f, se_r = 0.f;
  const int total = B * ld_xr;
  for (int i = blockIdx.x * 256 + threadIdx.x; i < total; i += gridDim.x * 256) {
    const int b = i / ld_xr, c = i - b * ld_xr;
    float g = 0.f;
    if (c < S) {
      const float d = xr[i] - next_state[(size_t)b * ld_rec + c];
      se_s = fmaf(d, d, se_s);
      g = d * gs;
    } else if (c == S) {
      const float d = xr[i] - reward[(size_t)b * ld_rec];
      se_r = fmaf(d, d, se_r);
      g = d * gr;
    }
    dxr[i] = g;
  }
  se_s = block_sum<256>(se_s, scratch);
  se_r = block_sum<256>(se_r, scratch);
  if (threadIdx.x == 0) {
    partial[2 * blockIdx.x] = se_s;
    partial[2 * blockIdx.x + 1] = se_r;
  }
}

__global__ void __launch_bounds__(256) vae_kl_bwd_kernel(const float* __restrict__ enc_head,
                                                         const float* __restrict__ prior_head, int ld_head, int B, int D,
                                                         const float* __restrict__ eps, const float* __restrict__ dz,
                                                         float* __restrict__ d_enc, float* __restrict__ d_prior,
                                                         float* __restrict__ partial) {
  __shared__ float scratch[33];
  const int total = B * D;
  const float g = 1.f / (float)total;
  float kl_sum = 0.f;
  for (int i = blockIdx.x * 256 + threadIdx.x; i < total; i += gridDim.x * 256) {
    const int b = i / D, d = i - b * D;
    const float* he = enc_head + (size_t)b * ld_head;
// ... 286 lines not shown
  td_critic_loss_kernel<<<1, 256, 0, s>>>(reward, done, ld_rd, nq1, nq2, logp2, q1, q2, B, norm_B > 0 ? norm_B : B, gamma,
                                          c, dq1, dq2, metrics);
  RLREP_LAUNCHED("td_critic_loss", s);
}

void launch_actor_alpha_loss(const float* q1, const float* q2, const float* logp, int B, float target_entropy,
                             int learn_alpha, Control* c, float* dq1, float* dq2, float* dlogp_scalar, float* metrics,
                             cudaStream_t s) {
  actor_alpha_loss_kernel<<<1, 256, 0, s>>>(q1, q2, logp, B, target_entropy, learn_alpha, c, dq1, dq2, dlogp_scalar,
                                            metrics);
  RLREP_LAUNCHED("actor_alpha_loss", s);
}

void launch_actor_loss_partial(const float* q1, const float* q2, const float* logp, int B, int norm_B,
                               float target_entropy, const Control* c, float* dq1, float* dq2, float* dlogp_scalar,
                               float* partial, cudaStream_t s) {
  actor_loss_partial_kernel<<<1, 256, 0, s>>>(q1, q2, logp, B, norm_B, target_entropy, c, dq1, dq2, dlogp_scalar, partial);
  RLREP_LAUNCHED("actor_loss_partial", s);
}
void launch_alpha_step(const float* reduced, int learn_alpha, Control* c, float* metrics, cudaStream_t s) {
  alpha_step_kernel<<<1, 32, 0, s>>>(reduced, learn_alpha, c, metrics);
  RLREP_LAUNCHED("alpha_step", s);
}
void launch_mul_dact(float* x, const float* aux, size_t n, int dact, cudaStream_t s) {
  mul_dact_kernel<<<grid_for(n, 256), 256, 0, s>>>(x, aux, n, dact);
  RLREP_LAUNCHED_W("mul_dact", s, 12.0 * (double)n, 0.0);
}

void launch_pack_columns(const float* in, int ld_in, float* out, int ld_out, int rows, const ColSegment* segs, int n_segs,
                         cudaStream_t s) {
  RLREP_CHECK(n_segs >= 1 && n_segs <= 3, "pack_columns takes 1..3 segments");
  ColSegments cs;
  cs.n = n_segs;
  int width = 0;
  for (int i = 0; i < n_segs; ++i) {
    cs.s[i] = segs[i];
    width += segs[i].len;
  }
  pack_columns_kernel<<<grid_for((size_t)rows * width, 256), 256, 0, s>>>(in, ld_in, out, ld_out, rows, cs, width);
  RLREP_LAUNCHED("pack_columns", s);
}
void launch_vae_sample(const float* head, int ld_head, int B, int D, const float* eps, float* z, cudaStream_t s) {
  vae_sample_kernel<<<grid_for((size_t)B * D, 256), 256, 0, s>>>(head, ld_head, B, D, eps, z);
  RLREP_LAUNCHED("vae_sample", s);
}
void launch_vae_recon_loss(const float* xr, int ld_xr, const float* next_state, const float* reward, int ld_rec, int B,
                           int S, float* dxr, float* partial, int n_blocks, cudaStream_t s) {
  vae_recon_loss_kernel<<<n_blocks, 256, 0, s>>>(xr, ld_xr, next_state, reward, ld_rec, B, S, dxr, partial);
  RLREP_LAUNCHED("vae_recon_loss", s);
}
void launch_vae_kl_bwd(const float* enc_head, const float* prior_head, int ld_head, int B, int D, const float* eps,
                       const float* dz, float* d_enc, float* d_prior, float* partial, int n_blocks, cudaStream_t s) {
  vae_kl_bwd_kernel<<<n_blocks, 256, 0, s>>>(enc_head, prior_head, ld_head, B, D, eps, dz, d_enc, d_prior, partial);
  RLREP_LAUNCHED("vae_kl_bwd", s);
}
void launch_vae_finalize(const float* recon_partial, int n_recon, const float* kl_partial, int n_kl, int B, int S, int D,
                         float* metrics, cudaStream_t s) {
  vae_finalize_kernel<<<1, 32, 0, s>>>(recon_partial, n_recon, kl_partial, n_kl, B, S, D, metrics);
  RLREP_LAUNCHED("vae_finalize", s);
}
void launch_noise_expand(const float* head, int ld_head, int B, int D, const float* noise, int NN, float* x,
                         cudaStream_t s) {
  const bool vec = (D & 3) == 0 && (ld_head & 3) == 0 && (long long)B * NN * D < (1LL << 31) &&
                   ((reinterpret_cast<uintptr_t>(head) | reinterpret_cast<uintptr_t>(noise) | reinterpret_cast<uintptr_t>(x)) & 15) == 0;
  if (vec) noise_expand4_kernel<<<grid_for((size_t)B * (D / 4), 256, 16), 256, 0, s>>>(head, ld_head, B, D, noise, NN, x);
  else noise_expand_kernel<<<grid_for((size_t)B * NN * D, 256, 16), 256, 0, s>>>(head, ld_head, B, D, noise, NN, x);
  RLREP_LAUNCHED("noise_expand", s);
}
void launch_noise_expand_bwd(const float* dx, const float* head, int ld_head, int B, int D, const float* noise, int NN,
                             float* d_head, cudaStream_t s) {
  noise_expand_bwd_kernel<<<grid_for((size_t)B * D, 256), 256, 0, s>>>(dx, head, ld_head, B, D, noise, NN, d_head);
  RLREP_LAUNCHED("noise_expand_bwd", s);
}
void launch_group_mean(const float* hid, int ld, int B, int NN, int C, float* out, cudaStream_t s) {
  group_mean_kernel<<<grid_for((size_t)B * C, 256), 256, 0, s>>>(hid, ld, B, NN, C, out);
  RLREP_LAUNCHED("group_mean", s);
}
void launch_group_mean_bwd(const float* dmean, const float* hid, int ld, int B, int NN, int C, float* dhid,
                           float* colsum_partial, cudaStream_t s) {
  group_mean_bwd_kernel<<<grid_for((size_t)B * C, 256), 256, 0, s>>>(dmean, hid, ld, B, NN, C, dhid, colsum_partial);
  RLREP_LAUNCHED("group_mean_bwd", s);
}

void launch_adam_polyak(float* p, const float* g, float* m, float* v, size_t n, const AdamHyper* hyper, float* target,
                        size_t n_polyak, float tau, const int* polyak_flag, cudaStream_t s) {
  RLREP_CHECK(n % 4 == 0 && n_polyak % 4 == 0, "optimizer arenas are padded to float4");
  const size_t n4 = n / 4;
  launch_pdl(adam_polyak_kernel, grid_for(n4, 256, 16), 256, 0, s, reinterpret_cast<float4*>(p),
             reinterpret_cast<const float4*>(g), reinterpret_cast<float4*>(m), reinterpret_cast<float4*>(v), n4, hyper,
             reinterpret_cast<float4*>(target), n_polyak / 4, tau, polyak_flag);
  const double polyak = target ? 12.0 * (double)n_polyak * (polyak_flag ? 0.5 : 1.0) : 0.0;
  RLREP_LAUNCHED_W("adam_polyak", s, 28.0 * (double)n + polyak, 0.0);
}

void launch_polyak(const float* p, float* target, size_t n, float tau, const int* polyak_flag, cudaStream_t s) {
  RLREP_CHECK(n % 4 == 0, "optimizer arenas are padded to float4");
  polyak_kernel<<<grid_for(n / 4, 256, 16), 256, 0, s>>>(reinterpret_cast<const float4*>(p),
                                                        reinterpret_cast<float4*>(target), n / 4, tau, polyak_flag);
  RLREP_LAUNCHED_W("polyak", s, 12.0 * (double)n * (polyak_flag ? 0.5 : 1.0), 0.0);
}

}
```

rlrep_b200/csrc/kernels.cuh:

```cuda
#pragma once
#include <cuda_runtime.h>

#include <cstdint>

#include "epilogue.cuh"

namespace rlrep {

constexpr int kMaxFeatureSteps = 16;
constexpr int kNumMetrics = 32;

struct AdamHyper {
  float step_size;
  float bc2_sqrt;
};

struct Control {
  int steps;
  int polyak_critic;
  long long t_feat, t_critic, t_actor, t_alpha;
  AdamHyper feat[kMaxFeatureSteps];
  AdamHyper critic, actor;
  double alpha_step_size, alpha_bc2_sqrt;
  double log_alpha, la_m, la_v;
  float alpha;
};

struct TickParams {
  int k_feat;
  int period;
  double lr_feat, lr_critic, lr_actor, lr_alpha;
  int critic_steps;
};

void launch_tick(Control* c, const TickParams& p, cudaStream_t s);

void launch_gather(const float* ring, int rec4, const long long* idx, int B, float* out, cudaStream_t s);
void launch_ring_write(float* ring, int rec4, long long capacity, long long start, const float* rows, int n,
                       cudaStream_t s);

void launch_ce_rows(float* logits, int ld, int rows, int cols, int diag_off, float inv_batch, float* loss_rows,
                    cudaStream_t s);

void launch_rowdot(const float* X, int ld, int rows, int D, const float* w, const float* b, float* y, cudaStream_t s);
struct RowDotJob {
  const float* X;
  const float* w;
  const float* b;
  float* y;
  int ld, D;
};
void launch_rowdot_pair(const RowDotJob& a, const RowDotJob& b, int rows, cudaStream_t s);
void launch_colreduce(const float* X, int ld, int rows, int cols, const float* u, float* out, int accumulate,
                      cudaStream_t s);
void launch_kgroup_finish(const float* ws, int groups, int M, int N, int ldw, size_t group_stride, float* C, int ldc,
                          const Epilogue& epi, cudaStream_t s);
void launch_colsum_finish(const float* partial, int chunks, int cols, float* out, cudaStream_t s);
void launch_colsum_tall(const float* X, int ld, long long rows, int cols, float* partial, int chunks, float* out,
                        cudaStream_t s);
struct ColJob {
  const float* X;
  const float* u;
  float* out;
  int ld, rows, cols;
};
constexpr int kMaxColJobs = 8;
void launch_colreduce_multi(const ColJob* jobs, int n_jobs, cudaStream_t s);
void launch_outer_dact(const float* u, const float* w, int rows, int cols, const float* aux, int ld_aux, int dact,
                       float* out, int ld_out, cudaStream_t s);

void launch_feature_loss_finalize(const float* loss_rows, int rows, const float* pred, const float* reward, int ld_r,
                                  float inv_batch, float* dpred, float* metrics , cudaStream_t s);

void launch_actor_sample(const float* head, int ld_head, int B, int A, const float* eps, float* action, int lda,
                         float* logp, cudaStream_t s, const float* obs = nullptr, int ld_obs = 0, int S = 0);
struct ActorSampleJob {
  const float* head;
  const float* eps;
  float* action;
  float* logp;
  const float* obs;
  int ld_obs;
};
void launch_actor_sample_pair(const ActorSampleJob& j0, const ActorSampleJob& j1, int ld_head, int B, int A, int lda, int S,
                              cudaStream_t s);
void launch_contrastive_head(float* logits, int ld, int rows, int cols, int diag_off, float inv_batch, const float* z, int ldz,
                             int D, const float* theta_w, const float* theta_b, const float* reward, int ld_r,
                             float* loss_rows, float* pred, float* dpred, float* metrics, unsigned* counter,
                             cudaStream_t s);
void launch_actor_act(const float* in, int rows, int S, int A, int H, const float* W0, int ld0, const float* b0,
                      const float* W1, int ld1, const float* b1, const float* W2, int ld2, const float* b2, int explore,
                      float* out, cudaStream_t s);
void launch_actor_sample_bwd(const float* head, int ld_head, int B, int A, const float* eps, const float* d_action,
                             int ldd, const float* dlogp_scalar, float* dhead, int ld_dhead, cudaStream_t s);

void launch_td_critic_loss(const float* reward, const float* done, int ld_rd, const float* nq1, const float* nq2,
                           const float* logp2, const float* q1, const float* q2, int B, float gamma, const Control* c,
                           float* dq1, float* dq2, float* metrics, cudaStream_t s, int norm_B = 0);
// ... 49 lines not shown
                           int S, float* dxr, float* partial, int n_blocks, cudaStream_t s);
void launch_vae_kl_bwd(const float* enc_head, const float* prior_head, int ld_head, int B, int D, const float* eps,
                       const float* dz, float* d_enc, float* d_prior, float* partial, int n_blocks, cudaStream_t s);
void launch_vae_finalize(const float* recon_partial, int n_recon, const float* kl_partial, int n_kl, int B, int S, int D,
                         float* metrics, cudaStream_t s);
void launch_noise_expand(const float* head, int ld_head, int B, int D, const float* noise, int NN, float* x,
                         cudaStream_t s);
void launch_noise_expand_bwd(const float* dx, const float* head, int ld_head, int B, int D, const float* noise, int NN,
                             float* d_head, cudaStream_t s);
void launch_group_mean(const float* hid, int ld, int B, int NN, int C, float* out, cudaStream_t s);
void launch_group_mean_bwd(const float* dmean, const float* hid, int ld, int B, int NN, int C, float* dhid,
                           float* colsum_partial, cudaStream_t s);

void launch_speder_rows(const float* zphi, const float* zmu, int D, int B, const float* theta_w, const float* theta_b,
                        const float* u, float* diag, float* rpred, float* c, cudaStream_t s);
void launch_speder_finalize(const float* diag, const float* c, const float* rpred, const float* reward, int ld_r, int B,
                            float* drp, float* metrics, cudaStream_t s);
void launch_speder_grad(const float* zphi, const float* zmu, int D, int B, const float* drp, const float* theta_w,
                        const float* c, const float* u, const float* w, float* dzphi, float* dzmu, cudaStream_t s);

void launch_diffsr_perturb(const float* next_state, int ld_rec, const float* noise, const long long* level,
                           const float* alphabars, int n_levels, float sigma, int B, int S, float* xin, int ld_x,
                           float* target, float* coef, cudaStream_t s);
void launch_diffsr_score(const float* phi, const float* flat, int D, int S, const float* target, const float* coef, int B,
                         float* dscore, float* loss_rows, cudaStream_t s);
void launch_diffsr_score_bwd(const float* phi, const float* flat, int D, int S, int B, const float* dscore, float* dflat,
                             float* dphi, cudaStream_t s);
void launch_sum_scaled(const float* x, int n, float scale, float* out, cudaStream_t s);

void launch_ln_tanh_fwd(const float* x, int ld_x, int B, int n, const float* gamma, const float* beta, float* y, int ld_y,
                        float* xhat, int ld_h, float* rstd, cudaStream_t s);
void launch_ln_tanh_bwd(const float* dy, int ld_dy, const float* y, int ld_y, const float* xhat, int ld_h, const float* rstd,
                        int B, int n, const float* gamma, float* dx, int ld_dx, float* g_beta, float* g_gamma, int ld_g,
                        cudaStream_t s);
void launch_trunc_normal_sample(const float* raw, int ld_raw, int B, int A, const float* eps, float std, float clip,
                                float* mu, float* action, int ld_a, cudaStream_t s);
void launch_trunc_normal_bwd(const float* d_action, int ld_da, const float* mu, int B, int A, float* draw, int ld_out,
                             cudaStream_t s);
void launch_drq_critic_loss(const float* reward, const float* discount, const float* tq1, const float* tq2, const float* q1,
                            const float* q2, int B, float* dq1, float* dq2, float* metrics, cudaStream_t s);
void launch_drq_actor_loss(const float* q1, const float* q2, int B, float* dq1, float* dq2, float* metrics, cudaStream_t s);

void launch_ln_act_fwd(const float* x, int ld_x, int B, int n, const float* gamma, const float* beta, bool use_tanh,
                       float* y, int ld_y, int zero_to, float* xhat, int ld_h, float* rstd, cudaStream_t s);
void launch_ln_act_bwd(const float* dy, int ld_dy, const float* y, int ld_y, const float* xhat, int ld_h, const float* rstd,
                       int B, int n, const float* gamma, bool use_tanh, float* dx, int ld_dx, int zero_to, float* g_beta,
                       float* g_gamma, int ld_g, cudaStream_t s);
void launch_gauss_sample(const float* m, const float* raw, int ld, int B, int D, const float* eps, float* z, int ld_z,
                         cudaStream_t s);
void launch_gauss_kl_bwd(const float* m1, const float* raw1, const float* m2, const float* raw2, int ld, int B, int D,
                         const float* eps, const float* dz, float w, const float* dcm, const float* dcraw, float* dm1,
                         float* draw1, float* dm2, float* draw2, float* partial, int n_blocks, cudaStream_t s);
void launch_gauss_noise_expand(const float* m, const float* raw, int ld, int B, int D, const float* noise, int NN,
                               float c_noise, float* x, int ld_x, cudaStream_t s);
void launch_gauss_noise_expand_bwd(const float* dx, int ld_x, const float* raw, int ld, int B, int D, const float* noise,
                                   int NN, float c_noise, float* dm, float* draw, cudaStream_t s);
void launch_group_mean_bwd_dact(const float* dmean, const float* hid, int ld, int B, int NN, int C, int dact, float* dhid,
                                float* colsum_partial, cudaStream_t s);
void launch_huber_critic_loss(const float* reward, const float* discount, const float* tq1, const float* tq2,
                              const float* q1, const float* q2, int B, float* dq1, float* dq2, float* metrics,
                              cudaStream_t s);
void launch_reward_mse(const float* r_hat, const float* reward, int B, float w, float* dr, float* out, cudaStream_t s);

void launch_ln_act2_fwd(const float* x, int ld_x, int B, int n, const float* gamma, const float* beta, int act, float* y,
                        int ld_y, int zero_to, float* xhat, int ld_h, float* rstd, cudaStream_t s);
void launch_ln_act2_bwd(const float* dy, int ld_dy, const float* y, int ld_y, const float* xhat, int ld_h, const float* rstd,
                        int B, int n, const float* gamma, const float* beta, int act, float* dx, int ld_dx, int zero_to,
                        float* g_beta, float* g_gamma, int ld_g, cudaStream_t s);
void launch_mish_fwd(const float* x, size_t n, float* y, cudaStream_t s);
void launch_mish_bwd(const float* dy, const float* x, size_t n, float* dx, cudaStream_t s);
void launch_mask_scale(const float* x, const float* mask, float inv_keep, size_t n, int accumulate, float* out, cudaStream_t s);
void launch_posterior_fwd(const float* h, int N, int L, const float* eps, float* mean_out, float* z, float* partial,
                          int n_blocks, cudaStream_t s);
void launch_posterior_bwd(const float* h, int N, int L, const float* eps, const float* dz, const float* dmean_extra,
                          int n_extra, float w_kl, float* dh, cudaStream_t s);
void launch_ldiff_perturb(const float* x, const float* noise, const float* ab, const float* temb, int B, int L, int T,
                          float inv_feat, float* zin, int ld, float* target, float* coef, cudaStream_t s);
void launch_ldiff_perturb_bwd(const float* dzin, int ld, const float* ab, int B, int L, float* dx, cudaStream_t s);
void launch_add_inplace(float* y, const float* x, size_t n, cudaStream_t s);
void launch_scale_inplace(float* p, size_t n, float scale, cudaStream_t s);

void launch_adam_polyak(float* p, const float* g, float* m, float* v, size_t n, const AdamHyper* hyper, float* target,
                        size_t n_polyak, float tau, const int* polyak_flag, cudaStream_t s);
void launch_polyak(const float* p, float* target, size_t n, float tau, const int* polyak_flag, cudaStream_t s);

}
```

rlrep_b200/csrc/ptx.cuh:

```cuda
#pragma once
#include <cstdint>
#include <cuda.h>
#include <cuda_runtime.h>

namespace rlrep {
namespace ptx {

__device__ __forceinline__ uint32_t smem_u32(const void* p) {
  return static_cast<uint32_t>(__cvta_generic_to_shared(p));
}

__device__ __forceinline__ bool elect_one() {
  uint32_t pred = 0;
  asm volatile(
      "{\n"
      ".reg .b32 rx;\n"
      ".reg .pred px;\n"
      "elect.sync rx|px, 0xffffffff;\n"
      "selp.u32 %0, 1, 0, px;\n"
      "}\n"
      : "=r"(pred));
  return pred != 0;
}

__device__ __forceinline__ void pdl_wait() { asm volatile("griddepcontrol.wait;" ::: "memory"); }
__device__ __forceinline__ void pdl_launch_dependents() { asm volatile("griddepcontrol.launch_dependents;" ::: "memory"); }

__device__ __forceinline__ void mbar_init(uint64_t* bar, uint32_t count) {
  asm volatile("mbarrier.init.shared::cta.b64 [%0], %1;" ::"r"(smem_u32(bar)), "r"(count) : "memory");
}
__device__ __forceinline__ void fence_mbar_init() {
  asm volatile("fence.mbarrier_init.release.cluster;" ::: "memory");
}
__device__ __forceinline__ void fence_proxy_async_smem() {
  asm volatile("fence.proxy.async.shared::cta;" ::: "memory");
}
__device__ __forceinline__ void mbar_arrive_expect_tx(uint64_t* bar, uint32_t bytes) {
  asm volatile("mbarrier.arrive.expect_tx.shared::cta.b64 _, [%0], %1;" ::"r"(smem_u32(bar)), "r"(bytes)
               : "memory");
}
__device__ __forceinline__ void mbar_arrive(uint64_t* bar) {
  asm volatile("mbarrier.arrive.shared::cta.b64 _, [%0];" ::"r"(smem_u32(bar)) : "memory");
}
__device__ __forceinline__ bool mbar_try_wait(uint64_t* bar, uint32_t parity) {
  uint32_t ok;
  asm volatile(
      "{\n"
      ".reg .pred p;\n"
      "mbarrier.try_wait.parity.shared::cta.b64 p, [%1], %2;\n"
      "selp.u32 %0, 1, 0, p;\n"
      "}\n"
      : "=r"(ok)
      : "r"(smem_u32(bar)), "r"(parity)
      : "memory");
  return ok != 0;
}
__device__ __forceinline__ void mbar_wait(uint64_t* bar, uint32_t parity) {
  if (mbar_try_wait(bar, parity)) return;
  const long long t0 = clock64();
  while (!mbar_try_wait(bar, parity)) {
    if (clock64() - t0 > 4000000000LL) {
      printf("rlrep: mbarrier wait timed out (block %d,%d,%d thread %d)\n", blockIdx.x, blockIdx.y,
             blockIdx.z, threadIdx.x);
      __trap();
    }
  }
}

__device__ __forceinline__ void prefetch_tensormap(const CUtensorMap* m) {
  asm volatile("prefetch.tensormap [%0];" ::"l"(reinterpret_cast<uint64_t>(m)) : "memory");
}
__device__ __forceinline__ void tma_load_2d(void* smem_dst, const CUtensorMap* m, uint64_t* bar, int c_inner,
                                            int c_outer) {
  asm volatile(
      "cp.async.bulk.tensor.2d.shared::cluster.global.mbarrier::complete_tx::bytes [%0], [%1, {%3, %4}], [%2];"
      ::"r"(smem_u32(smem_dst)),
      "l"(reinterpret_cast<uint64_t>(m)), "r"(smem_u32(bar)), "r"(c_inner), "r"(c_outer)
      : "memory");
}
__device__ __forceinline__ void tma_load_3d(void* smem_dst, const CUtensorMap* m, uint64_t* bar, int c0, int c1, int c2) {
  asm volatile(
      "cp.async.bulk.tensor.3d.shared::cluster.global.mbarrier::complete_tx::bytes [%0], [%1, {%3, %4, %5}], [%2];"
      ::"r"(smem_u32(smem_dst)),
      "l"(reinterpret_cast<uint64_t>(m)), "r"(smem_u32(bar)), "r"(c0), "r"(c1), "r"(c2)
      : "memory");
}
__device__ __forceinline__ void tma_load_4d(void* smem_dst, const CUtensorMap* m, uint64_t* bar, int c0, int c1, int c2,
                                            int c3) {
  asm volatile(
      "cp.async.bulk.tensor.4d.shared::cluster.global.mbarrier::complete_tx::bytes [%0], [%1, {%3, %4, %5, %6}], [%2];"
      ::"r"(smem_u32(smem_dst)),
      "l"(reinterpret_cast<uint64_t>(m)), "r"(smem_u32(bar)), "r"(c0), "r"(c1), "r"(c2), "r"(c3)
      : "memory");
}
__device__ __forceinline__ void bulk_load_1d(void* smem_dst, const void* gsrc, uint32_t bytes, uint64_t* bar) {
  asm volatile(
      "cp.async.bulk.shared::cluster.global.mbarrier::complete_tx::bytes [%0], [%1], %2, [%3];" ::"r"(
          smem_u32(smem_dst)),
      "l"(reinterpret_cast<uint64_t>(gsrc)), "r"(bytes), "r"(smem_u32(bar))
      : "memory");
}

__device__ __forceinline__ void tmem_alloc(uint32_t* smem_result, uint32_t ncols) {
  asm volatile("tcgen05.alloc.cta_group::1.sync.aligned.shared::cta.b32 [%0], %1;" ::"r"(smem_u32(smem_result)),
               "r"(ncols)
               : "memory");
}
__device__ __forceinline__ void tmem_relinquish() {
  asm volatile("tcgen05.relinquish_alloc_permit.cta_group::1.sync.aligned;" ::: "memory");
}
__device__ __forceinline__ void tmem_dealloc(uint32_t taddr, uint32_t ncols) {
  asm volatile("tcgen05.dealloc.cta_group::1.sync.aligned.b32 %0, %1;" ::"r"(taddr), "r"(ncols) : "memory");
}
__device__ __forceinline__ void tc_fence_before_sync() {
  asm volatile("tcgen05.fence::before_thread_sync;" ::: "memory");
}
__device__ __forceinline__ void tc_fence_after_sync() {
  asm volatile("tcgen05.fence::after_thread_sync;" ::: "memory");
}
__device__ __forceinline__ void mma_tf32_ss(uint32_t tmem_d, uint64_t adesc, uint64_t bdesc, uint32_t idesc,
                                            uint32_t accumulate) {
  asm volatile(
      "{\n"
      ".reg .pred p;\n"
      "setp.ne.b32 p, %4, 0;\n"
      "tcgen05.mma.cta_group::1.kind::tf32 [%0], %1, %2, %3, p;\n"
      "}\n" ::"r"(tmem_d),
      "l"(adesc), "l"(bdesc), "r"(idesc), "r"(accumulate)
      : "memory");
}
__device__ __forceinline__ void mma_commit(uint64_t* bar) {
  asm volatile("tcgen05.commit.cta_group::1.mbarrier::arrive::one.shared::cluster.b64 [%0];" ::"r"(smem_u32(bar))
               : "memory");
}
__device__ __forceinline__ void tmem_ld_32x32b_x32(uint32_t taddr, uint32_t (&r)[32]) {
  asm volatile(
      "tcgen05.ld.sync.aligned.32x32b.x32.b32 "
      "{%0, %1, %2, %3, %4, %5, %6, %7, %8, %9, %10, %11, %12, %13, %14, %15, "
      "%16, %17, %18, %19, %20, %21, %22, %23, %24, %25, %26, %27, %28, %29, %30, %31}, [%32];"
      : "=r"(r[0]), "=r"(r[1]), "=r"(r[2]), "=r"(r[3]), "=r"(r[4]), "=r"(r[5]), "=r"(r[6]), "=r"(r[7]),
        "=r"(r[8]), "=r"(r[9]), "=r"(r[10]), "=r"(r[11]), "=r"(r[12]), "=r"(r[13]), "=r"(r[14]), "=r"(r[15]),
        "=r"(r[16]), "=r"(r[17]), "=r"(r[18]), "=r"(r[19]), "=r"(r[20]), "=r"(r[21]), "=r"(r[22]), "=r"(r[23]),
        "=r"(r[24]), "=r"(r[25]), "=r"(r[26]), "=r"(r[27]), "=r"(r[28]), "=r"(r[29]), "=r"(r[30]), "=r"(r[31])
      : "r"(taddr)
      : "memory");
}
__device__ __forceinline__ void tmem_ld_32x32b_x16(uint32_t taddr, uint32_t (&r)[16]) {
  asm volatile(
      "tcgen05.ld.sync.aligned.32x32b.x16.b32 "
      "{%0, %1, %2, %3, %4, %5, %6, %7, %8, %9, %10, %11, %12, %13, %14, %15}, [%16];"
      : "=r"(r[0]), "=r"(r[1]), "=r"(r[2]), "=r"(r[3]), "=r"(r[4]), "=r"(r[5]), "=r"(r[6]), "=r"(r[7]),
        "=r"(r[8]), "=r"(r[9]), "=r"(r[10]), "=r"(r[11]), "=r"(r[12]), "=r"(r[13]), "=r"(r[14]), "=r"(r[15])
      : "r"(taddr)
      : "memory");
}
__device__ __forceinline__ void tmem_ld_wait() { asm volatile("tcgen05.wait::ld.sync.aligned;" ::: "memory"); }

__device__ __forceinline__ void cluster_sync() {
  asm volatile("barrier.cluster.arrive.release.aligned;\n\tbarrier.cluster.wait.acquire.aligned;" ::: "memory");
}
__device__ __forceinline__ void cluster_arrive() {
  asm volatile("barrier.cluster.arrive.release.aligned;" ::: "memory");
}
__device__ __forceinline__ void cluster_arrive_relaxed() {
  asm volatile("barrier.cluster.arrive.relaxed.aligned;" ::: "memory");
}
__device__ __forceinline__ void cluster_wait() {
  asm volatile("barrier.cluster.wait.acquire.aligned;" ::: "memory");
}
__device__ __forceinline__ uint32_t cluster_ctarank() {
  uint32_t r;
  asm volatile("mov.u32 %0, %%cluster_ctarank;" : "=r"(r));
  return r;
}
__device__ __forceinline__ float4 ld_shared_f4(uint32_t addr) {
  float4 v;
  asm volatile("ld.shared.v4.f32 {%0, %1, %2, %3}, [%4];" : "=f"(v.x), "=f"(v.y), "=f"(v.z), "=f"(v.w) : "r"(addr) : "memory");
  return v;
}
__device__ __forceinline__ void st_dsmem_f4(uint32_t addr, uint32_t cta_rank, float4 v) {
  uint32_t remote;
  asm volatile("mapa.shared::cluster.u32 %0, %1, %2;" : "=r"(remote) : "r"(addr), "r"(cta_rank));
  asm volatile("st.shared::cluster.v4.f32 [%0], {%1, %2, %3, %4};" ::"r"(remote), "f"(v.x), "f"(v.y), "f"(v.z), "f"(v.w)
               : "memory");
// ... 31 lines not shown
```

rlrep_b200/csrc/runtime.cu:

```cuda
#include <algorithm>
#include <atomic>

#include "agent.cuh"

namespace rlrep {

namespace {
thread_local long long g_launches = 0;
thread_local bool g_profiling = false;
thread_local std::vector<cudaEvent_t> g_events;
thread_local std::vector<const char*> g_names;
thread_local std::vector<double> g_bytes, g_flops;
}

long long launch_count() { return g_launches; }

void note_launch(const char* name, cudaStream_t stream, double bytes, double flops) {
  if (std::strncmp(name, "nccl_", 5) != 0) ++g_launches;
  if (g_profiling) {
    cudaEvent_t e;
    if (cudaEventCreate(&e) == cudaSuccess) {
      cudaEventRecord(e, stream);
      g_events.push_back(e);
      g_names.push_back(name);
// ... 58 lines not shown
  RLREP_CUDA(cudaMallocHost(&idx_host_, idx_cap_ * sizeof(long long)));
  RLREP_CUDA(cudaMalloc(&idx_dev_, idx_cap_ * sizeof(long long)));
}

Ring::~Ring() {
  cudaFree(data);
  cudaFreeHost(stage_host_);
  cudaFree(stage_dev_);
  cudaFreeHost(idx_host_);
  cudaFree(idx_dev_);
}

void Ring::add_packed(const float* rows_host, int n, cudaStream_t s) {
  int done = 0;
  while (done < n) {
    const int chunk = (int)std::min<size_t>(std::min<size_t>(stage_rows_, (size_t)capacity), (size_t)(n - done));
    RLREP_CUDA(cudaStreamSynchronize(s));
    std::memcpy(stage_host_, rows_host + (size_t)done * R, (size_t)chunk * R * sizeof(float));
    RLREP_CUDA(cudaMemcpyAsync(stage_dev_, stage_host_, (size_t)chunk * R * sizeof(float), cudaMemcpyHostToDevice, s));
    launch_ring_write(data, R / 4, capacity, ptr, stage_dev_, chunk, s);
    ptr = (ptr + chunk) % capacity;
    size = std::min(size + chunk, capacity);
    done += chunk;
  }
  RLREP_CUDA(cudaStreamSynchronize(s));
}

void Ring::load_columns(const void* state, const void* action, const void* next_state, const void* reward,
                        const void* done, long long n, int is_f64, cudaStream_t s) {
  RLREP_CHECK(n <= capacity, "more rows than ring capacity");
  auto get = [is_f64](const void* base, long long i) -> float {
    return is_f64 ? (float)static_cast<const double*>(base)[i] : static_cast<const float*>(base)[i];
  };
  ptr = 0;
  size = 0;
  long long row = 0;
  while (row < n) {
    const int chunk = (int)std::min<long long>((long long)stage_rows_, n - row);
    RLREP_CUDA(cudaStreamSynchronize(s));
    std::memset(stage_host_, 0, (size_t)chunk * R * sizeof(float));
    for (int i = 0; i < chunk; ++i) {
      float* rec = stage_host_ + (size_t)i * R;
      const long long r = row + i;
      for (int j = 0; j < S; ++j) rec[j] = get(state, r * S + j);
      for (int j = 0; j < A; ++j) rec[off_a + j] = get(action, r * A + j);
      rec[off_r] = get(reward, r);
      rec[off_d] = get(done, r);
      for (int j = 0; j < S; ++j) rec[off_s2 + j] = get(next_state, r * S + j);
    }
    RLREP_CUDA(cudaMemcpyAsync(stage_dev_, stage_host_, (size_t)chunk * R * sizeof(float), cudaMemcpyHostToDevice, s));
    launch_ring_write(data, R / 4, capacity, ptr, stage_dev_, chunk, s);
    ptr = (ptr + chunk) % capacity;
    size = std::min(size + chunk, capacity);
    row += chunk;
  }
  RLREP_CUDA(cudaStreamSynchronize(s));
}

void Ring::gather_from_host_idx(const long long* idx_host, int B, float* out_dev, cudaStream_t s) {
  RLREP_CHECK(B > 0 && B <= idx_cap_, "batch too large for the ring's index staging");
  for (int i = 0; i < B; ++i) RLREP_CHECK(idx_host[i] >= 0 && idx_host[i] < size, "replay index out of range");
  RLREP_CUDA(cudaStreamSynchronize(s));
  std::memcpy(idx_host_, idx_host, (size_t)B * sizeof(long long));
  RLREP_CUDA(cudaMemcpyAsync(idx_dev_, idx_host_, (size_t)B * sizeof(long long), cudaMemcpyHostToDevice, s));
  launch_gather(data, R / 4, idx_dev_, B, out_dev, s);
}

void GemmRunner::init(Precision prec, size_t ws_floats) {
  prec_ = prec;
  ws_floats_ = ws_floats;
  if (ws_floats_) RLREP_CUDA(cudaMalloc(&ws_, ws_floats_ * sizeof(float)));
}
GemmRunner::~GemmRunner() {
  if (ws_) cudaFree(ws_);
  if (kg_ws_) cudaFree(kg_ws_);
}

void GemmRunner::begin_chain(cudaStream_t s) {
  RLREP_CHECK(!recording_, "begin_chain inside a chain");
  if (!chains_enabled()) return;
  recording_ = true;
  chain_stream_ = s;
  pending_.clear();
}

void GemmRunner::flush_chain() {
  if (pending_.empty()) return;
  if (pending_.size() == 1) {
    const GemmArgs a = pending_[0];
    pending_.clear();
    const bool rec = recording_;
    recording_ = false;
    run(a, chain_stream_);
    recording_ = rec;
    return;
  }
  GemmChain* chain = nullptr;
  for (auto& c : chains_)
    if (c->matches(pending_)) chain = c.get();
  if (chain == nullptr) {
    chains_.emplace_back(new GemmChain());
    chain = chains_.back().get();
    chain->build(pending_);
  }
  chain->launch(chain_stream_);
  pending_.clear();
}

void GemmRunner::end_chain() {
  if (!recording_) return;
  flush_chain();
  recording_ = false;
}

bool GemmRunner::compact_supported(GemmArgs a, int wp, int ho) {
  if (recording_ || prec_ != PREC_TF32 || !tc_eligible(a) || a.conv_w <= 0 || a.M < 32 || a.N != 32 || wp <= 8 ||
      a.M >= (1 << 24))
    return false;
  a.compact_wp = wp;
  a.compact_ho = ho;
  const TcGemmPlan probe = make_tc_plan(a, 0, 0, ws_, ws_floats_, sm_share_);
  return probe.halo_rows > 0;
}
bool GemmRunner::run_compact(GemmArgs a, int wp, int ho, cudaStream_t s) {
  if (!compact_supported(a, wp, ho)) return false;
  a.compact_wp = wp;
  a.compact_ho = ho;
  run(a, s);
  return true;
}

void GemmRunner::run(const GemmArgs& a, cudaStream_t s) {
  if (recording_) {
    if (chain_eligible(a)) {
      pending_.push_back(a);
      return;
    }
    flush_chain();
    s = chain_stream_;
  }
  const bool tc = prec_ == PREC_TF32 && tc_eligible(a) && a.M >= 32 && a.N >= 32 && a.K >= 8;
  RLREP_CHECK(a.compact_wp == 0 || tc, "compacting stores exist on the tensor-core halo kernel only");
  if (!tc) {
    launch_simt(a, s);
    return;
  }
  if (a.k_groups == 1 && a.conv_w == 0 && a.conv_wgrad_hi == 0 && !recording_) {
    const int tiles = ceil_div(a.M, 128) * ceil_div(a.N, 128), nkb = ceil_div(a.K, 32);
    int groups = 1;
    constexpr int kCtaCap = 296;
    while (groups < 8 && tiles * 8 * groups * 2 <= kCtaCap && nkb >= 256 * groups * 2) groups *= 2;
    if (groups > 1 && nkb >= 1024) {
      const int ldw = (a.N + 3) & ~3, m_pad = ceil_div(a.M, 128) * 128;
      const size_t need = (size_t)groups * m_pad * ldw;
      if (need > kg_ws_floats_) {
        cudaStreamCaptureStatus cap = cudaStreamCaptureStatusNone;
        RLREP_CUDA(cudaStreamIsCapturing(s, &cap));
        RLREP_CHECK(cap == cudaStreamCaptureStatusNone, "K-group workspace must be sized before a graph capture");
        if (kg_ws_) RLREP_CUDA(cudaFree(kg_ws_));
        RLREP_CUDA(cudaMalloc(&kg_ws_, need * sizeof(float)));
        kg_ws_floats_ = need;
        plans_.clear();
      }
      GemmArgs g = a;
      g.C = kg_ws_; g.ldc = ldw;
      g.epi = Epilogue();
      g.k_groups = groups;
      run(g, s);
      launch_kgroup_finish(kg_ws_, groups, a.M, a.N, ldw, (size_t)m_pad * ldw, a.C, a.ldc, a.epi, s);
      return;
    }
  }
  std::string key(sizeof(GemmArgs), '\0');
  {
    GemmArgs* k = reinterpret_cast<GemmArgs*>(&key[0]);
    k->M = a.M; k->N = a.N; k->K = a.K;
    k->A = a.A; k->lda = a.lda; k->a_mn = a.a_mn;
    k->B = a.B; k->ldb = a.ldb; k->b_mn = a.b_mn;
    k->C = a.C; k->ldc = a.ldc; k->conv_w = a.conv_w; k->conv_wgrad_hi = a.conv_wgrad_hi;
    k->compact_wp = a.compact_wp; k->compact_ho = a.compact_ho; k->k_groups = a.k_groups;
    k->compact_hx = a.compact_hx; k->compact_stride = a.compact_stride; k->compact_oy = a.compact_oy;
    k->compact_ox = a.compact_ox; k->compact_out_w = a.compact_out_w; k->conv_ntaps = a.conv_ntaps;
    for (int t = 0; t < 9; ++t) { k->conv_tap_shift[t] = a.conv_tap_shift[t]; k->conv_tap_kb[t] = a.conv_tap_kb[t]; }
    k->epi.bias = a.epi.bias; k->epi.r1_u = a.epi.r1_u; k->epi.r1_v = a.epi.r1_v; k->epi.aux = a.epi.aux;
    k->epi.pre_out = a.epi.pre_out; k->epi.ld_aux = a.epi.ld_aux; k->epi.ld_pre = a.epi.ld_pre;
    k->epi.act = a.epi.act; k->epi.dact = a.epi.dact; k->epi.accumulate = a.epi.accumulate;
    k->epi.scale = a.epi.scale;
    k->K1 = sm_share_ < 0.75 ? 1 : 0;
  }
  auto it = plans_.find(key);
  if (it == plans_.end()) it = plans_.emplace(key, make_tc_plan(a, 0, 0, ws_, ws_floats_, sm_share_)).first;
  launch_tc(it->second, s);
}

void linear_fwd(GemmRunner& g, cudaStream_t s, int rows, Mat x, const Linear& l, int act, float* y, int ldy, Mat x2,
                int k1, float* pre_out) {
  GemmArgs a;
  const bool pad_n = l.out < 32 && l.out_alloc >= 32 && ldy >= l.out_alloc && rows >= 64 && pre_out == nullptr;
  a.M = rows; a.N = pad_n ? l.out_alloc : l.out; a.K = l.in;
  a.A = x.p; a.lda = x.ld;
  if (x2.p) { a.A2 = x2.p; a.lda2 = x2.ld; a.K1 = k1; }
  a.B = l.W; a.ldb = l.ld;
  a.C = y; a.ldc = ldy;
  a.epi.bias = l.b;
  a.epi.act = act;
  if (pre_out) { a.epi.pre_out = pre_out; a.epi.ld_pre = ldy; }
  g.run(a, s);
}

void linear_dgrad(GemmRunner& g, cudaStream_t s, int rows, Mat dy, const Linear& l, int dact, Mat aux, float* dx,
                  int lddx, int col0, int n_cols) {
  GemmArgs a;
  a.M = rows; a.N = n_cols < 0 ? l.in : n_cols; a.K = l.out;
  a.A = dy.p; a.lda = dy.ld;
  a.B = l.W + col0; a.ldb = l.ld; a.b_mn = true;
  a.C = dx; a.ldc = lddx;
// ... 95 lines not shown
```

Before: 1316.

## Fuse Adam updates for chained weight slots into the persistent GEMM chain kernel

Adds Adam/Polyak optimiser tasks to the persistent GEMM chain kernel. The producer warp bulk-loads p, g, m and v chunks into shared memory with an evict-first hint, and the epilogue warps run the update once the weight-gradient GEMMs that task depends on have finished. In the ctrlsac feature step, four weight slots are updated this way, and the standalone Adam kernel now covers only the remaining ranges through a multi-range variant. The intent is to overlap the optimiser with the tail of the GEMM chain and cut Adam memory traffic and launch latency after the chain. The cost is extra dependency tracking, a per-element range lookup in the Adam kernel, and pipeline stages shared between GEMM and Adam tasks.

```diff
diff --git a/include/rlrep_b200.h b/include/rlrep_b200.h
--- a/include/rlrep_b200.h
+++ b/include/rlrep_b200.h
@@ -57,6 +57,11 @@
 RLREP_EXPORT int rlrep_gemm_chain_add(int M, int N, int K, const float* A_dev, int lda, int a_mn, const float* B_dev,
                                       int ldb, int b_mn, float* C_dev, int ldc, const rlrep_epilogue* epi);
 RLREP_EXPORT int rlrep_gemm_chain_run(void* stream, int bn, int split_k, int iters, float* ms_out, int* levels_out);
+RLREP_EXPORT int rlrep_gemm_chain_add_adam(float* p_dev, const float* g_dev, float* m_dev, float* v_dev, size_t n,
+                                           const float* hyper_dev, float* target_dev, float tau, const int* polyak_flag_dev);
+RLREP_EXPORT int rlrep_adam_polyak(void* stream, float* p_dev, const float* g_dev, float* m_dev, float* v_dev, size_t n,
+                                   const float* hyper_dev, float* target_dev, size_t n_polyak, float tau,
+                                   const int* polyak_flag_dev);
 RLREP_EXPORT int rlrep_gemm_chain_set_debug(unsigned long long* dev);
 
 RLREP_EXPORT int rlrep_gemm_trace(unsigned long long* out16_host);
diff --git a/rlrep_b200/_lib.py b/rlrep_b200/_lib.py
--- a/rlrep_b200/_lib.py
+++ b/rlrep_b200/_lib.py
@@ -76,6 +76,8 @@
         "rlrep_gemm_chain_set_debug": [vp],
         "rlrep_gemm_chain_add": [i, i, i, vp, i, i, vp, i, i, vp, i, C.POINTER(Epilogue)],
         "rlrep_gemm_chain_run": [vp, i, i, i, C.POINTER(C.c_float), C.POINTER(C.c_int)],
+        "rlrep_gemm_chain_add_adam": [vp, vp, vp, vp, sz, vp, vp, f, vp],
+        "rlrep_adam_polyak": [vp, vp, vp, vp, vp, sz, vp, vp, sz, f, vp],
         "rlrep_ring_create": [i, i, C.c_longlong, C.POINTER(vp)],
         "rlrep_ring_destroy": [vp],
         "rlrep_ring_layout": [vp] + [C.POINTER(i)] * 5,
@@ -229,9 +231,17 @@
     return C_out
 
 
-def gemm_chain(specs, *, bn=0, split_k=0, iters=1):
+def _ptr(t):
+    return t.data_ptr() if t is not None else None
+
+
+def gemm_chain(specs, *, bn=0, split_k=0, iters=1, adam=()):
     lib = load()
     check(lib.rlrep_gemm_chain_begin())
+    for a in adam:
+        check(lib.rlrep_gemm_chain_add_adam(a["p"].data_ptr(), a["g"].data_ptr(), a["m"].data_ptr(), a["v"].data_ptr(),
+                                            a["p"].numel(), a["hyper"].data_ptr(), _ptr(a.get("target")),
+                                            float(a.get("tau", 0.0)), _ptr(a.get("polyak_flag"))))
     keep = []
     for A, B, C_out, kw in specs:
         a_mn, b_mn = bool(kw.get("a_mn", False)), bool(kw.get("b_mn", False))
@@ -248,6 +258,11 @@
     return ms.value, levels.value
 
 
+def adam_polyak(p, g, m, v, hyper, *, target=None, n_polyak=0, tau=0.0, polyak_flag=None):
+    check(load().rlrep_adam_polyak(current_stream_ptr(), p.data_ptr(), g.data_ptr(), m.data_ptr(), v.data_ptr(),
+                                   p.numel(), hyper.data_ptr(), _ptr(target), n_polyak, float(tau), _ptr(polyak_flag)))
+
+
 def gemm_bench(A, B, C_out, *, a_mn=False, b_mn=False, path="tc", epi=None, bn=0, split_k=0, ws=None, iters=50):
     lib = load()
     M = A.shape[1] if a_mn else A.shape[0]
diff --git a/rlrep_b200/csrc/agent.cuh b/rlrep_b200/csrc/agent.cuh
--- a/rlrep_b200/csrc/agent.cuh
+++ b/rlrep_b200/csrc/agent.cuh
@@ -197,12 +197,14 @@
   void begin_chain(cudaStream_t s);
   void end_chain();
   bool recording() const { return recording_; }
+  bool chain_adam(const ChainAdamArgs& a);
 
  private:
   void flush_chain();
   bool recording_ = false;
   cudaStream_t chain_stream_ = nullptr;
   std::vector<GemmArgs> pending_;
+  std::vector<ChainAdamArgs> pending_adam_;
   std::vector<std::unique_ptr<GemmChain>> chains_;
   Precision prec_ = PREC_TF32;
   double sm_share_ = 1.0;
diff --git a/rlrep_b200/csrc/agent_ctrlsac.cu b/rlrep_b200/csrc/agent_ctrlsac.cu
--- a/rlrep_b200/csrc/agent_ctrlsac.cu
+++ b/rlrep_b200/csrc/agent_ctrlsac.cu
@@ -273,6 +273,22 @@
     linear_wgrad(gemm_, s0, B_, Mat{dg2_, H_}, Mat{g1_, H_}, n2, Mat(), 0, false);
     linear_wgrad(gemm_, s0, B_, Mat{dh1_, H_}, sa(), l1, Mat(), 0, false);
     linear_wgrad(gemm_, s0, B_, Mat{dg1_, H_}, s2(), n1, Mat(), 0, false);
+    const LinearSlot* in_chain[4] = {&p2_, &p3_, &m2_, &m3_};
+    bool chained_adam = true;
+    for (const LinearSlot* w : in_chain) {
+      ChainAdamArgs a;
+      a.p = feat_g_.p + w->w_off;
+      a.g = feat_g_.g + w->w_off;
+      a.m = feat_g_.m + w->w_off;
+      a.v = feat_g_.v + w->w_off;
+      a.n = w->b_off - w->w_off;
+      a.hyper = &ctl->feat[k];
+      if (cfg.use_feature_target && w->w_off < feat_g_.n_target) {
+        a.target = feat_g_.target + w->w_off;
+        a.tau = cfg.feature_tau;
+      }
+      chained_adam = gemm_.chain_adam(a);
+    }
     gemm_.end_chain();
     {
       ColJob jobs[8] = {bias_job(B_, Mat{dzphi_, D_}, l3), bias_job(B_, Mat{dh2_, H_}, l2),
@@ -282,9 +298,19 @@
                         bias_job(B_, Mat{dg1_, H_}, n1)};
       launch_colreduce_multi(jobs, 8, s0);
     }
-    launch_adam_polyak(feat_g_.p, feat_g_.g, feat_g_.m, feat_g_.v, feat_g_.n, &ctl->feat[k],
-                       cfg.use_feature_target ? feat_g_.target : nullptr, feat_g_.n_target, cfg.feature_tau, nullptr,
-                       s0);
+    AdamRange rest[5];
+    int n_rest = 0;
+    size_t from = 0;
+    if (chained_adam) {
+      for (const LinearSlot* w : in_chain) {
+        rest[n_rest++] = AdamRange{from, w->w_off};
+        from = w->b_off;
+      }
+    }
+    rest[n_rest++] = AdamRange{from, feat_g_.n};
+    launch_adam_polyak_ranges(feat_g_.p, feat_g_.g, feat_g_.m, feat_g_.v, rest, n_rest, &ctl->feat[k],
+                              cfg.use_feature_target ? feat_g_.target : nullptr, feat_g_.n_target, cfg.feature_tau,
+                              nullptr, s0);
   }
 
   void critic_step_chained() {
diff --git a/rlrep_b200/csrc/capi.cu b/rlrep_b200/csrc/capi.cu
--- a/rlrep_b200/csrc/capi.cu
+++ b/rlrep_b200/csrc/capi.cu
@@ -143,6 +143,7 @@
 
 namespace {
 thread_local std::vector<GemmArgs> g_chain_seq;
+thread_local std::vector<ChainAdamArgs> g_chain_adam;
 }
 
 int rlrep_gemm_chain_set_debug(unsigned long long* dev) {
@@ -154,6 +155,26 @@
 int rlrep_gemm_chain_begin(void) {
   RLREP_API_BEGIN
   g_chain_seq.clear();
+  g_chain_adam.clear();
+  RLREP_API_END
+}
+
+int rlrep_gemm_chain_add_adam(float* p, const float* g, float* m, float* v, size_t n, const float* hyper, float* target,
+                              float tau, const int* polyak_flag) {
+  RLREP_API_BEGIN
+  ChainAdamArgs a;
+  a.p = p; a.g = g; a.m = m; a.v = v; a.n = n;
+  a.hyper = reinterpret_cast<const AdamHyper*>(hyper);
+  a.target = target; a.tau = tau; a.polyak_flag = polyak_flag;
+  g_chain_adam.push_back(a);
+  RLREP_API_END
+}
+
+int rlrep_adam_polyak(void* stream, float* p, const float* g, float* m, float* v, size_t n, const float* hyper,
+                      float* target, size_t n_polyak, float tau, const int* polyak_flag) {
+  RLREP_API_BEGIN
+  launch_adam_polyak(p, g, m, v, n, reinterpret_cast<const AdamHyper*>(hyper), target, n_polyak, tau, polyak_flag,
+                     static_cast<cudaStream_t>(stream));
   RLREP_API_END
 }
 
@@ -176,7 +197,7 @@
   RLREP_CHECK(!g_chain_seq.empty() && iters >= 1, "empty chain");
   cudaStream_t st = static_cast<cudaStream_t>(stream);
   GemmChain chain;
-  chain.build(g_chain_seq, bn, split_k);
+  chain.build(g_chain_seq, g_chain_adam, bn, split_k);
   if (levels_out) *levels_out = chain.levels();
   cudaEvent_t e0, e1;
   RLREP_CUDA(cudaEventCreate(&e0));
@@ -192,6 +213,7 @@
   cudaEventDestroy(e1);
   if (ms_out) *ms_out = iters > 1 ? ms / (iters - 1) : 0.f;
   g_chain_seq.clear();
+  g_chain_adam.clear();
   RLREP_API_END
 }
 
diff --git a/rlrep_b200/csrc/gemm_chain.cu b/rlrep_b200/csrc/gemm_chain.cu
--- a/rlrep_b200/csrc/gemm_chain.cu
+++ b/rlrep_b200/csrc/gemm_chain.cu
@@ -163,9 +163,9 @@
 }
 
 __global__ void __launch_bounds__(kThreads, 1)
-gemm_chain_kernel(const ChainGemmDesc* __restrict__ gemms, const ChainTask* __restrict__ tasks,
-                  const int* __restrict__ task_begin, unsigned* __restrict__ done, unsigned* __restrict__ exit_ctr,
-                  int n_gemms, unsigned long long* __restrict__ dbg) {
+gemm_chain_kernel(const ChainGemmDesc* __restrict__ gemms, const ChainAdamDesc* __restrict__ adams,
+                  const ChainTask* __restrict__ tasks, const int* __restrict__ task_begin, unsigned* __restrict__ done,
+                  unsigned* __restrict__ exit_ctr, int n_gemms, unsigned long long* __restrict__ dbg) {
   auto stamp = [&](int item, int ev) {
     if (dbg != nullptr && item < kDbgItems) {
       unsigned long long t;
@@ -211,8 +211,37 @@
   if (warp == 0) {
     if (lane == 0) {
       int it = 0, last_gemm = -1;
+      uint64_t evict_first = 0;
       for (int t = t_begin; t < t_end; ++t) {
         const ChainTask tk = tasks[t];
+        if (tk.adam) {
+          const ChainAdamDesc* a = adams + tk.gemm;
+          const int n_deps = a->n_deps;
+          const int off = tk.tile * kChainAdamChunk;
+          const uint32_t bytes = 4u * (uint32_t)min(kChainAdamChunk, a->n - off);
+          stamp(t - t_begin, 0);
+          if (dbg != nullptr && t - t_begin < kDbgItems)
+            dbg[((size_t)blockIdx.x * kDbgItems + (t - t_begin)) * kDbgEvents + 8] =
+                (unsigned long long)tk.gemm | ((unsigned long long)tk.tile << 16) | (1ull << 62);
+          for (int d = 0; d < n_deps; ++d) wait_counter(done, a->dep[d], (int)a->dep_target[d]);
+          if (n_deps > 0) {
+            fence_acquire_gpu();
+            fence_proxy_async_global();
+          }
+          stamp(t - t_begin, 1);
+          if (evict_first == 0) evict_first = ptx::policy_evict_first();
+          const int s = it % kStages;
+          ptx::mbar_wait(&empty_bar[s], ((it / kStages) & 1) ^ 1);
+          ptx::mbar_arrive_expect_tx(&full_bar[s], 4 * bytes);
+          float* dst = reinterpret_cast<float*>(smem + s * kStageBytes);
+          ptx::bulk_load_1d(dst, a->p + off, bytes, &full_bar[s]);
+          ptx::bulk_load_1d_hint(dst + kChainAdamChunk, a->g + off, bytes, &full_bar[s], evict_first);
+          ptx::bulk_load_1d_hint(dst + 2 * kChainAdamChunk, a->m + off, bytes, &full_bar[s], evict_first);
+          ptx::bulk_load_1d_hint(dst + 3 * kChainAdamChunk, a->v + off, bytes, &full_bar[s], evict_first);
+          ++it;
+          stamp(t - t_begin, 2);
+          continue;
+        }
         const ChainGemmDesc* g = gemms + tk.gemm;
         const int n_deps = g->n_deps;
         const int bn = g->bn, a_mn = g->a_mn, b_mn = g->b_mn;
@@ -260,8 +289,9 @@
   } else if (warp == 1) {
     if (ptx::elect_one()) {
       int it = 0, tc = 0;
-      for (int t = t_begin; t < t_end; ++t, ++tc) {
+      for (int t = t_begin; t < t_end; ++t) {
         const ChainTask tk = tasks[t];
+        if (tk.adam) break;
         const ChainGemmDesc* g = gemms + tk.gemm;
         const int bn = g->bn, a_mn = g->a_mn, b_mn = g->b_mn;
         const int kb0 = tk.split * g->kb_per_split, kb1 = min(g->nkb, kb0 + g->kb_per_split);
@@ -289,14 +319,16 @@
         }
         ptx::mma_commit(&acc_full[acc]);
         stamp(t - t_begin, 4);
+        ++tc;
       }
     }
   } else {
     const int q = warp & 3, half = (warp - 2) >> 2;
     float* tw = tbuf + (warp - 2) * (32 * kTwPitch);
-    int tc = 0;
-    for (int t = t_begin; t < t_end; ++t, ++tc) {
+    int tc = 0, t = t_begin;
+    for (; t < t_end; ++t, ++tc) {
       const ChainTask tk = tasks[t];
+      if (tk.adam) break;
       const ChainGemmDesc* g = gemms + tk.gemm;
       const Epilogue epi = g->epi;
       const int bn = g->bn, M = g->M, N = g->N, ldc = g->ldc, split_k = g->split_k;
@@ -466,6 +498,55 @@
       __syncwarp();
       if (lane == 0) ptx::mbar_arrive(&acc_empty[acc]);
     }
+    for (; t < t_end; ++t) {
+      const ChainTask tk = tasks[t];
+      const ChainAdamDesc* a = adams + tk.gemm;
+      const int e = threadIdx.x - 64;
+      const int off = tk.tile * kChainAdamChunk;
+      const int n4 = min(kChainAdamChunk, a->n - off) / 4;
+      float4* p = reinterpret_cast<float4*>(a->p + off);
+      float4* m = reinterpret_cast<float4*>(a->m + off);
+      float4* v = reinterpret_cast<float4*>(a->v + off);
+      float4* target = reinterpret_cast<float4*>(a->target + off);
+      const bool do_polyak = a->target != nullptr && (a->polyak_flag == nullptr || *a->polyak_flag != 0);
+      const float ss = a->hyper->step_size, bc2s = a->hyper->bc2_sqrt, tau = a->tau, omt = 1.f - tau;
+      const int s = tk.split % kStages;
+      float4 tv[2];
+#pragma unroll
+      for (int j = 0; j < 2; ++j)
+        if (do_polyak && e + 256 * j < n4) tv[j] = __ldcs(target + e + 256 * j);
+      ptx::mbar_wait(&full_bar[s], (tk.split / kStages) & 1);
+      if (threadIdx.x == 64) stamp(t - t_begin, 5);
+      const float4* st = reinterpret_cast<const float4*>(smem + s * kStageBytes);
+#pragma unroll
+      for (int j = 0; j < 2; ++j) {
+        const int i = e + 256 * j;
+        if (i < n4) {
+          float4 pv = st[i], mv = st[kChainAdamChunk / 2 + i], vv = st[3 * kChainAdamChunk / 4 + i];
+          const float4 gv = st[kChainAdamChunk / 4 + i];
+          adam_elem(pv.x, gv.x, mv.x, vv.x, ss, bc2s);
+          adam_elem(pv.y, gv.y, mv.y, vv.y, ss, bc2s);
+          adam_elem(pv.z, gv.z, mv.z, vv.z, ss, bc2s);
+          adam_elem(pv.w, gv.w, mv.w, vv.w, ss, bc2s);
+          p[i] = pv;
+          __stcs(m + i, mv);
+          __stcs(v + i, vv);
+          if (do_polyak) {
+            float4 tt = tv[j];
+            tt.x = polyak_elem(pv.x, tt.x, tau, omt);
+            tt.y = polyak_elem(pv.y, tt.y, tau, omt);
+            tt.z = polyak_elem(pv.z, tt.z, tau, omt);
+            tt.w = polyak_elem(pv.w, tt.w, tau, omt);
+            __stcs(target + i, tt);
+          }
+        }
+      }
+      epilogue_bar();
+      if (threadIdx.x == 64) {
+        ptx::mbar_arrive(&empty_bar[s]);
+        stamp(t - t_begin, 7);
+      }
+    }
   }
   ptx::pdl_launch_dependents();
   ptx::tc_fence_before_sync();
@@ -509,6 +590,16 @@
   f.writes.push_back(range_of(a.epi.pre_out, a.M, a.epi.ld_pre, a.N));
   return f;
 }
+Footprint footprint(const ChainAdamArgs& a) {
+  Footprint f;
+  const long long n = (long long)a.n;
+  for (const float* x : {(const float*)a.p, (const float*)a.m, (const float*)a.v, (const float*)a.target}) {
+    f.reads.push_back(range_of(x, 1, 0, n));
+    f.writes.push_back(range_of(x, 1, 0, n));
+  }
+  f.reads.push_back(range_of(a.g, 1, 0, n));
+  return f;
+}
 bool conflicts(const Footprint& earlier, const Footprint& later) {
   for (const Range& w : earlier.writes) {
     for (const Range& r : later.reads)
@@ -521,6 +612,8 @@
       if (w.overlaps(r)) return true;
   return false;
 }
+
+bool aligned16_host(const void* p) { return (reinterpret_cast<uintptr_t>(p) & 15) == 0; }
 
 unsigned long long* g_chain_dbg = nullptr;
 
@@ -557,8 +650,14 @@
   if (dev_) cudaFree(dev_);
 }
 
-bool GemmChain::matches(const std::vector<GemmArgs>& seq) const {
-  if (seq.size() != seq_.size()) return false;
+bool GemmChain::matches(const std::vector<GemmArgs>& seq, const std::vector<ChainAdamArgs>& adam) const {
+  if (seq.size() != seq_.size() || adam.size() != adam_.size()) return false;
+  for (size_t i = 0; i < adam.size(); ++i) {
+    const ChainAdamArgs &x = adam[i], &y = adam_[i];
+    if (x.p != y.p || x.g != y.g || x.m != y.m || x.v != y.v || x.n != y.n || x.hyper != y.hyper || x.target != y.target ||
+        x.tau != y.tau || x.polyak_flag != y.polyak_flag)
+      return false;
+  }
   for (size_t i = 0; i < seq.size(); ++i) {
     const GemmArgs &x = seq[i], &y = seq_[i];
     if (x.M != y.M || x.N != y.N || x.K != y.K || x.A != y.A || x.B != y.B || x.C != y.C || x.lda != y.lda ||
@@ -571,12 +670,21 @@
   return true;
 }
 
-void GemmChain::build(const std::vector<GemmArgs>& seq, int force_bn, int force_split) {
+void GemmChain::build(const std::vector<GemmArgs>& seq, const std::vector<ChainAdamArgs>& adam, int force_bn,
+                      int force_split) {
   RLREP_CHECK(dev_ == nullptr, "chain already built");
   RLREP_CHECK(!seq.empty(), "empty chain");
-  const int n = (int)seq.size();
+  const int n = (int)seq.size(), na = (int)adam.size();
   for (const GemmArgs& a : seq) RLREP_CHECK(chain_eligible(a), "GEMM cannot be a member of a chain");
+  for (const ChainAdamArgs& a : adam) {
+    RLREP_CHECK(a.p && a.g && a.m && a.v && a.hyper && a.n > 0 && a.n % 4 == 0 && a.n < (1u << 30),
+                "chain optimiser item: p, g, m, v, hyper and a length that is a positive multiple of 4");
+    RLREP_CHECK(aligned16_host(a.p) && aligned16_host(a.g) && aligned16_host(a.m) && aligned16_host(a.v) &&
+                    aligned16_host(a.target),
+                "chain optimiser item: 16-byte aligned tensors");
+  }
   seq_ = seq;
+  adam_ = adam;
   int n_sm = kNumSMs;
   {
     int dev = 0;
@@ -617,6 +725,28 @@
     RLREP_CHECK((int)deps[j].size() <= kChainMaxDeps, "a chain GEMM has too many direct dependencies");
   }
   levels_ = 1 + *std::max_element(level.begin(), level.end());
+  std::vector<Footprint> fpa(na);
+  std::vector<std::vector<int>> adeps(na);
+  std::vector<int> alevel(na, 0);
+  for (int x = 0; x < na; ++x) {
+    fpa[x] = footprint(adam[x]);
+    for (int y = 0; y < x; ++y) RLREP_CHECK(!conflicts(fpa[y], fpa[x]), "chain optimiser items overlap");
+    std::vector<int> direct;
+    const Range tgt = range_of(adam[x].target, 1, 0, (long long)adam[x].n);
+    for (int i = 0; i < n; ++i) {
+      for (const Range& w : fp[i].writes)
+        RLREP_CHECK(!w.overlaps(tgt), "a chain GEMM writes the Polyak target of an optimiser item");
+      if (conflicts(fp[i], fpa[x])) direct.push_back(i);
+    }
+    for (int i : direct) {
+      bool implied = false;
+      for (int k : direct)
+        if (k != i && reach[k][i]) implied = true;
+      if (!implied) adeps[x].push_back(i);
+      alevel[x] = std::max(alevel[x], level[i] + 1);
+    }
+    RLREP_CHECK((int)adeps[x].size() <= kChainMaxDeps, "a chain optimiser item has too many direct dependencies");
+  }
 
   std::vector<int> bn(n), split(n), share(n), first_cta(n), dist(n, 0);
   const int dist_mode = env_int("RLREP_CHAIN_DIST", 1);
@@ -712,10 +842,47 @@
     bytes_ += 4.0 * ((double)a.M * a.K + (double)a.N * a.K + (double)a.M * a.N);
     flops_ += 2.0 * a.M * a.N * a.K;
   }
+  std::vector<ChainAdamDesc> adescs(na);
+  if (na > 0) {
+    std::vector<int> cta_order(n_cta), aorder(na);
+    for (int c = 0; c < n_cta; ++c) cta_order[c] = c;
+    std::stable_sort(cta_order.begin(), cta_order.end(),
+                     [&](int x, int y) { return per_cta[x].size() < per_cta[y].size(); });
+    for (int x = 0; x < na; ++x) aorder[x] = x;
+    std::stable_sort(aorder.begin(), aorder.end(), [&](int x, int y) { return alevel[x] < alevel[y]; });
+    int next = 0;
+    for (int x : aorder) {
+      const ChainAdamArgs& a = adam[x];
+      const int chunks = ceil_div((int)a.n, kChainAdamChunk);
+      for (int c = 0; c < chunks; ++c, ++next) per_cta[cta_order[next % n_cta]].push_back(ChainTask{x, c, 0, 1});
+      ChainAdamDesc& d = adescs[x];
+      std::memset(&d, 0, sizeof(d));
+      d.p = a.p; d.g = a.g; d.m = a.m; d.v = a.v; d.target = a.target;
+      d.hyper = a.hyper; d.polyak_flag = a.polyak_flag; d.tau = a.tau;
+      d.n = (int)a.n;
+      d.n_deps = (int)adeps[x].size();
+      for (int k = 0; k < d.n_deps; ++k) {
+        const int j = adeps[x][k];
+        d.dep[k] = j;
+        d.dep_target[k] = (unsigned)items_of(j);
+      }
+      bytes_ += 28.0 * (double)a.n + (a.target ? 12.0 * (double)a.n : 0.0);
+    }
+  }
   std::vector<ChainTask> tasks;
   std::vector<int> begin(n_cta + 1, 0);
   for (int c = 0; c < n_cta; ++c) {
     begin[c] = (int)tasks.size();
+    int it = 0;
+    for (ChainTask& tk : per_cta[c]) {
+      if (tk.adam) {
+        tk.split = it++;
+      } else {
+        const int kb_per = ceil_div(ceil_div(seq[tk.gemm].K, kBK), split[tk.gemm]);
+        const int nkb = ceil_div(seq[tk.gemm].K, kBK);
+        it += std::min(nkb, (tk.split + 1) * kb_per) - tk.split * kb_per;
+      }
+    }
     tasks.insert(tasks.end(), per_cta[c].begin(), per_cta[c].end());
   }
   begin[n_cta] = (int)tasks.size();
@@ -723,7 +890,8 @@
 
   auto up = [](size_t x) { return (x + 255) & ~size_t(255); };
   const size_t o_desc = 0;
-  const size_t o_tasks = up(o_desc + sizeof(ChainGemmDesc) * n);
+  const size_t o_adam = up(o_desc + sizeof(ChainGemmDesc) * n);
+  const size_t o_tasks = up(o_adam + sizeof(ChainAdamDesc) * na);
   const size_t o_begin = up(o_tasks + sizeof(ChainTask) * tasks.size());
   const size_t o_done = up(o_begin + sizeof(int) * begin.size());
   const size_t o_exit = up(o_done + sizeof(unsigned) * n * kSub * kCtrStride);
@@ -734,6 +902,7 @@
   RLREP_CUDA(cudaMemset(dev_, 0, o_ws));
   char* base = static_cast<char*>(dev_);
   d_gemms_ = reinterpret_cast<ChainGemmDesc*>(base + o_desc);
+  d_adam_ = na > 0 ? reinterpret_cast<ChainAdamDesc*>(base + o_adam) : nullptr;
   d_tasks_ = reinterpret_cast<ChainTask*>(base + o_tasks);
   d_task_begin_ = reinterpret_cast<int*>(base + o_begin);
   d_done_ = reinterpret_cast<unsigned*>(base + o_done);
@@ -743,6 +912,7 @@
     descs[i].ws = split[i] > 1 ? reinterpret_cast<float*>(base + o_ws) + ws_off[i] : nullptr;
   }
   RLREP_CUDA(cudaMemcpy(d_gemms_, descs.data(), sizeof(ChainGemmDesc) * n, cudaMemcpyHostToDevice));
+  if (na > 0) RLREP_CUDA(cudaMemcpy(d_adam_, adescs.data(), sizeof(ChainAdamDesc) * na, cudaMemcpyHostToDevice));
   RLREP_CUDA(cudaMemcpy(d_tasks_, tasks.data(), sizeof(ChainTask) * tasks.size(), cudaMemcpyHostToDevice));
   RLREP_CUDA(cudaMemcpy(d_task_begin_, begin.data(), sizeof(int) * begin.size(), cudaMemcpyHostToDevice));
   RLREP_CUDA(cudaDeviceSynchronize());
@@ -753,6 +923,9 @@
       std::fprintf(stderr, "  [%d] L%d M=%d N=%d K=%d a_mn=%d b_mn=%d bn=%d split=%d%s share=%d deps=%d\n", i, level[i],
                    seq[i].M, seq[i].N, seq[i].K, (int)seq[i].a_mn, (int)seq[i].b_mn, bn[i], split[i],
                    dist[i] ? " (distributed)" : "", share[i], (int)deps[i].size());
+    for (int x = 0; x < na; ++x)
+      std::fprintf(stderr, "  adam[%d] L%d n=%zu chunks=%d polyak=%d deps=%d\n", x, alevel[x], adam[x].n,
+                   ceil_div((int)adam[x].n, kChainAdamChunk), adam[x].target != nullptr, (int)adeps[x].size());
   }
 }
 
@@ -769,7 +942,8 @@
   attr[1] = pdl_attribute();
   cfg.attrs = attr;
   cfg.numAttrs = 2;
-  RLREP_CUDA(cudaLaunchKernelEx(&cfg, gemm_chain_kernel, (const ChainGemmDesc*)d_gemms_, (const ChainTask*)d_tasks_,
+  RLREP_CUDA(cudaLaunchKernelEx(&cfg, gemm_chain_kernel, (const ChainGemmDesc*)d_gemms_, (const ChainAdamDesc*)d_adam_,
+                                (const ChainTask*)d_tasks_,
                                 (const int*)d_task_begin_, d_done_, d_exit_, (int)seq_.size(), g_chain_dbg));
   RLREP_LAUNCHED_W("gemm_chain", stream, bytes_, flops_);
 }
diff --git a/rlrep_b200/csrc/gemm_chain.cuh b/rlrep_b200/csrc/gemm_chain.cuh
--- a/rlrep_b200/csrc/gemm_chain.cuh
+++ b/rlrep_b200/csrc/gemm_chain.cuh
@@ -2,6 +2,7 @@
 #include <vector>
 
 #include "gemm.cuh"
+#include "kernels.cuh"
 
 namespace rlrep {
 
@@ -23,8 +24,33 @@
   unsigned dep_target[kChainMaxDeps];
 };
 
+struct ChainAdamArgs {
+  float* p = nullptr;
+  const float* g = nullptr;
+  float *m = nullptr, *v = nullptr;
+  size_t n = 0;
+  const AdamHyper* hyper = nullptr;
+  float* target = nullptr;
+  float tau = 0.f;
+  const int* polyak_flag = nullptr;
+};
+constexpr int kChainAdamChunk = 2048;
+
+struct ChainAdamDesc {
+  float* p;
+  const float* g;
+  float *m, *v, *target;
+  const AdamHyper* hyper;
+  const int* polyak_flag;
+  float tau;
+  int n;
+  int n_deps;
+  int dep[kChainMaxDeps];
+  unsigned dep_target[kChainMaxDeps];
+};
+
 struct ChainTask {
-  int gemm, tile, split, pad;
+  int gemm, tile, split, adam;
 };
 
 class GemmChain {
@@ -33,16 +59,19 @@
   GemmChain(const GemmChain&) = delete;
   GemmChain& operator=(const GemmChain&) = delete;
   ~GemmChain();
-  bool matches(const std::vector<GemmArgs>& seq) const;
-  void build(const std::vector<GemmArgs>& seq, int force_bn = 0, int force_split = 0);
+  bool matches(const std::vector<GemmArgs>& seq, const std::vector<ChainAdamArgs>& adam = {}) const;
+  void build(const std::vector<GemmArgs>& seq, const std::vector<ChainAdamArgs>& adam = {}, int force_bn = 0,
+             int force_split = 0);
   void launch(cudaStream_t stream);
   int size() const { return (int)seq_.size(); }
   int levels() const { return levels_; }
 
  private:
   std::vector<GemmArgs> seq_;
+  std::vector<ChainAdamArgs> adam_;
   void* dev_ = nullptr;
   ChainGemmDesc* d_gemms_ = nullptr;
+  ChainAdamDesc* d_adam_ = nullptr;
   ChainTask* d_tasks_ = nullptr;
   int* d_task_begin_ = nullptr;
   unsigned* d_done_ = nullptr;
diff --git a/rlrep_b200/csrc/kernels.cu b/rlrep_b200/csrc/kernels.cu
--- a/rlrep_b200/csrc/kernels.cu
+++ b/rlrep_b200/csrc/kernels.cu
@@ -1,3 +1,4 @@
+#include <algorithm>
 #include <cmath>
 
 #include "common.cuh"
@@ -734,17 +735,15 @@
     x[i] *= apply_dact(aux[i], dact);
 }
 
-__device__ __forceinline__ float adam_elem(float& p, float g, float& m, float& v, float ss, float bc2s) {
-  constexpr float w1 = (float)(1.0 - 0.9), b2 = 0.999f, w2 = (float)(1.0 - 0.999), eps = 1e-8f;
-  m = fmaf(w1, g - m, m);
-  v = fmaf(w2 * g, g, v * b2);
-  const float denom = sqrtf(v) / bc2s + eps;
-  p = p - ss * (m / denom);
-  return p;
-}
+struct AdamRanges4 {
+  size_t begin4[kAdamMaxRanges];
+  size_t cum4[kAdamMaxRanges + 1];
+  int count;
+};
 
 __global__ void __launch_bounds__(256) adam_polyak_kernel(float4* __restrict__ p, const float4* __restrict__ g,
-                                                          float4* __restrict__ m, float4* __restrict__ v, size_t n4,
+                                                          float4* __restrict__ m, float4* __restrict__ v,
+                                                          const __grid_constant__ AdamRanges4 rg,
                                                           const AdamHyper* __restrict__ hyper,
                                                           float4* __restrict__ target, size_t n4_polyak, float tau,
                                                           const int* __restrict__ polyak_flag) {
@@ -753,7 +752,11 @@
   const float ss = hyper->step_size, bc2s = hyper->bc2_sqrt;
   const bool do_polyak = target != nullptr && (polyak_flag == nullptr || *polyak_flag != 0);
   const float omt = 1.f - tau;
-  for (size_t i = (size_t)blockIdx.x * blockDim.x + threadIdx.x; i < n4; i += (size_t)gridDim.x * blockDim.x) {
+  const size_t n4 = rg.cum4[rg.count];
+  int r = 0;
+  for (size_t j = (size_t)blockIdx.x * blockDim.x + threadIdx.x; j < n4; j += (size_t)gridDim.x * blockDim.x) {
+    while (j >= rg.cum4[r + 1]) ++r;
+    const size_t i = rg.begin4[r] + (j - rg.cum4[r]);
     float4 pv = p[i], mv = __ldcs(m + i), vv = __ldcs(v + i);
     const float4 gv = __ldcs(g + i);
     adam_elem(pv.x, gv.x, mv.x, vv.x, ss, bc2s);
@@ -765,10 +768,10 @@
     __stcs(v + i, vv);
     if (do_polyak && i < n4_polyak) {
       float4 t = __ldcs(target + i);
-      t.x = __fadd_rn(__fmul_rn(tau, pv.x), __fmul_rn(omt, t.x));
-      t.y = __fadd_rn(__fmul_rn(tau, pv.y), __fmul_rn(omt, t.y));
-      t.z = __fadd_rn(__fmul_rn(tau, pv.z), __fmul_rn(omt, t.z));
-      t.w = __fadd_rn(__fmul_rn(tau, pv.w), __fmul_rn(omt, t.w));
+      t.x = polyak_elem(pv.x, t.x, tau, omt);
+      t.y = polyak_elem(pv.y, t.y, tau, omt);
+      t.z = polyak_elem(pv.z, t.z, tau, omt);
+      t.w = polyak_elem(pv.w, t.w, tau, omt);
       __stcs(target + i, t);
     }
   }
@@ -781,10 +784,10 @@
   for (size_t i = (size_t)blockIdx.x * blockDim.x + threadIdx.x; i < n4; i += (size_t)gridDim.x * blockDim.x) {
     const float4 pv = p[i];
     float4 t = target[i];
-    t.x = __fadd_rn(__fmul_rn(tau, pv.x), __fmul_rn(omt, t.x));
-    t.y = __fadd_rn(__fmul_rn(tau, pv.y), __fmul_rn(omt, t.y));
-    t.z = __fadd_rn(__fmul_rn(tau, pv.z), __fmul_rn(omt, t.z));
-    t.w = __fadd_rn(__fmul_rn(tau, pv.w), __fmul_rn(omt, t.w));
+    t.x = polyak_elem(pv.x, t.x, tau, omt);
+    t.y = polyak_elem(pv.y, t.y, tau, omt);
+    t.z = polyak_elem(pv.z, t.z, tau, omt);
+    t.w = polyak_elem(pv.w, t.w, tau, omt);
     target[i] = t;
   }
 }
@@ -1237,15 +1240,34 @@
   RLREP_LAUNCHED("group_mean_bwd", s);
 }
 
+void launch_adam_polyak_ranges(float* p, const float* g, float* m, float* v, const AdamRange* ranges, int count,
+                               const AdamHyper* hyper, float* target, size_t n_polyak, float tau, const int* polyak_flag,
+                               cudaStream_t s) {
+  RLREP_CHECK(count >= 1 && count <= kAdamMaxRanges && n_polyak % 4 == 0, "adam_polyak: 1..8 ranges");
+  AdamRanges4 rg = {};
+  rg.count = count;
+  double n = 0.0, n_pol = 0.0;
+  for (int r = 0; r < count; ++r) {
+    const AdamRange& x = ranges[r];
+    RLREP_CHECK(x.begin % 4 == 0 && x.end % 4 == 0 && x.begin < x.end, "optimizer arenas are padded to float4");
+    RLREP_CHECK(r == 0 || x.begin >= ranges[r - 1].end, "adam_polyak ranges must be ascending and disjoint");
+    rg.begin4[r] = x.begin / 4;
+    rg.cum4[r + 1] = rg.cum4[r] + (x.end - x.begin) / 4;
+    n += (double)(x.end - x.begin);
+    n_pol += (double)(std::min(x.end, n_polyak) - std::min(x.begin, n_polyak));
+  }
+  launch_pdl(adam_polyak_kernel, grid_for(rg.cum4[count], 256, 16), 256, 0, s, reinterpret_cast<float4*>(p),
+             reinterpret_cast<const float4*>(g), reinterpret_cast<float4*>(m), reinterpret_cast<float4*>(v), rg, hyper,
+             reinterpret_cast<float4*>(target), n_polyak / 4, tau, polyak_flag);
+  const double polyak = target ? 12.0 * n_pol * (polyak_flag ? 0.5 : 1.0) : 0.0;
+  RLREP_LAUNCHED_W("adam_polyak", s, 28.0 * n + polyak, 0.0);
+}
+
 void launch_adam_polyak(float* p, const float* g, float* m, float* v, size_t n, const AdamHyper* hyper, float* target,
                         size_t n_polyak, float tau, const int* polyak_flag, cudaStream_t s) {
   RLREP_CHECK(n % 4 == 0 && n_polyak % 4 == 0, "optimizer arenas are padded to float4");
-  const size_t n4 = n / 4;
-  launch_pdl(adam_polyak_kernel, grid_for(n4, 256, 16), 256, 0, s, reinterpret_cast<float4*>(p),
-             reinterpret_cast<const float4*>(g), reinterpret_cast<float4*>(m), reinterpret_cast<float4*>(v), n4, hyper,
-             reinterpret_cast<float4*>(target), n_polyak / 4, tau, polyak_flag);
-  const double polyak = target ? 12.0 * (double)n_polyak * (polyak_flag ? 0.5 : 1.0) : 0.0;
-  RLREP_LAUNCHED_W("adam_polyak", s, 28.0 * (double)n + polyak, 0.0);
+  const AdamRange all{0, n};
+  launch_adam_polyak_ranges(p, g, m, v, &all, 1, hyper, target, n_polyak, tau, polyak_flag, s);
 }
 
 void launch_polyak(const float* p, float* target, size_t n, float tau, const int* polyak_flag, cudaStream_t s) {
diff --git a/rlrep_b200/csrc/kernels.cuh b/rlrep_b200/csrc/kernels.cuh
--- a/rlrep_b200/csrc/kernels.cuh
+++ b/rlrep_b200/csrc/kernels.cuh
@@ -14,6 +14,17 @@
   float step_size;
   float bc2_sqrt;
 };
+
+__device__ __forceinline__ void adam_elem(float& p, float g, float& m, float& v, float ss, float bc2s) {
+  constexpr float w1 = (float)(1.0 - 0.9), b2 = 0.999f, w2 = (float)(1.0 - 0.999), eps = 1e-8f;
+  m = fmaf(w1, g - m, m);
+  v = fmaf(w2 * g, g, v * b2);
+  const float denom = sqrtf(v) / bc2s + eps;
+  p = p - ss * (m / denom);
+}
+__device__ __forceinline__ float polyak_elem(float p, float t, float tau, float omt) {
+  return __fadd_rn(__fmul_rn(tau, p), __fmul_rn(omt, t));
+}
 
 struct Control {
   int steps;
@@ -229,6 +240,13 @@
 
 void launch_adam_polyak(float* p, const float* g, float* m, float* v, size_t n, const AdamHyper* hyper, float* target,
                         size_t n_polyak, float tau, const int* polyak_flag, cudaStream_t s);
+constexpr int kAdamMaxRanges = 8;
+struct AdamRange {
+  size_t begin, end;
+};
+void launch_adam_polyak_ranges(float* p, const float* g, float* m, float* v, const AdamRange* ranges, int count,
+                               const AdamHyper* hyper, float* target, size_t n_polyak, float tau, const int* polyak_flag,
+                               cudaStream_t s);
 void launch_polyak(const float* p, float* target, size_t n, float tau, const int* polyak_flag, cudaStream_t s);
 
 }
diff --git a/rlrep_b200/csrc/ptx.cuh b/rlrep_b200/csrc/ptx.cuh
--- a/rlrep_b200/csrc/ptx.cuh
+++ b/rlrep_b200/csrc/ptx.cuh
@@ -100,6 +100,19 @@
       "l"(reinterpret_cast<uint64_t>(gsrc)), "r"(bytes), "r"(smem_u32(bar))
       : "memory");
 }
+__device__ __forceinline__ void bulk_load_1d_hint(void* smem_dst, const void* gsrc, uint32_t bytes, uint64_t* bar,
+                                                  uint64_t policy) {
+  asm volatile(
+      "cp.async.bulk.shared::cluster.global.mbarrier::complete_tx::bytes.L2::cache_hint [%0], [%1], %2, [%3], %4;" ::"r"(
+          smem_u32(smem_dst)),
+      "l"(reinterpret_cast<uint64_t>(gsrc)), "r"(bytes), "r"(smem_u32(bar)), "l"(policy)
+      : "memory");
+}
+__device__ __forceinline__ uint64_t policy_evict_first() {
+  uint64_t pol;
+  asm volatile("createpolicy.fractional.L2::evict_first.b64 %0, 1.0;" : "=l"(pol));
+  return pol;
+}
 
 __device__ __forceinline__ void tmem_alloc(uint32_t* smem_result, uint32_t ncols) {
   asm volatile("tcgen05.alloc.cta_group::1.sync.aligned.shared::cta.b32 [%0], %1;" ::"r"(smem_u32(smem_result)),
diff --git a/rlrep_b200/csrc/runtime.cu b/rlrep_b200/csrc/runtime.cu
--- a/rlrep_b200/csrc/runtime.cu
+++ b/rlrep_b200/csrc/runtime.cu
@@ -164,11 +164,18 @@
   recording_ = true;
   chain_stream_ = s;
   pending_.clear();
+  pending_adam_.clear();
+}
+
+bool GemmRunner::chain_adam(const ChainAdamArgs& a) {
+  if (!recording_ || pending_.empty()) return false;
+  pending_adam_.push_back(a);
+  return true;
 }
 
 void GemmRunner::flush_chain() {
   if (pending_.empty()) return;
-  if (pending_.size() == 1) {
+  if (pending_.size() == 1 && pending_adam_.empty()) {
     const GemmArgs a = pending_[0];
     pending_.clear();
     const bool rec = recording_;
@@ -179,14 +186,15 @@
   }
   GemmChain* chain = nullptr;
   for (auto& c : chains_)
-    if (c->matches(pending_)) chain = c.get();
+    if (c->matches(pending_, pending_adam_)) chain = c.get();
   if (chain == nullptr) {
     chains_.emplace_back(new GemmChain());
     chain = chains_.back().get();
-    chain->build(pending_);
+    chain->build(pending_, pending_adam_);
   }
   chain->launch(chain_stream_);
   pending_.clear();
+  pending_adam_.clear();
 }
 
 void GemmRunner::end_chain() {
@@ -214,6 +222,7 @@
 
 void GemmRunner::run(const GemmArgs& a, cudaStream_t s) {
   if (recording_) {
+    RLREP_CHECK(pending_adam_.empty(), "a GEMM recorded after the chain's optimiser items");
     if (chain_eligible(a)) {
       pending_.push_back(a);
       return;
```

Result: slower. 1170 (median of 6 runs) (-11.1%).
